# naver/dust3r

Measured on NVIDIA H100. Metric: image-pairs/sec (512x384, ViT-L/B+DPT), higher is better.
Workload: dtype bf16

## Files before the change

### dust3r_b200/_lib.py

```python
from __future__ import annotations

import ctypes as C
import os

from ._lib_fwd import Model

_HERE = os.path.dirname(os.path.abspath(__file__))
LIB_PATH = os.path.join(_HERE, 'libdust3r_b200.so')

_lib = None


class D3RError(RuntimeError):
    pass


class AlignDesc(C.Structure):
    _fields_ = [
        ('n_imgs', C.c_int32), ('n_edges', C.c_int32), ('n_entries', C.c_int32), ('n_chunks', C.c_int32),
        ('max_deg', C.c_int32), ('max_chunks', C.c_int32), ('chunk_px', C.c_int32), ('dist_l2', C.c_int32), ('norm_pw_scale', C.c_int32),
        ('tied_focal', C.c_int32), ('eval_only', C.c_int32),
        ('base_scale', C.c_float), ('pw_break', C.c_float), ('focal_break', C.c_float), ('adam_eps', C.c_float),
        ('beta1', C.c_float), ('beta2', C.c_float),
        ('img_hw', C.c_void_p), ('img_pix_off', C.c_void_p), ('img_ent_ptr', C.c_void_p),
        ('img_chunk_ptr', C.c_void_p), ('chunk_img', C.c_void_p),
        ('ent_edge', C.c_void_p), ('ent_obs_off', C.c_void_p), ('ent_coef', C.c_void_p), ('edge_ent', C.c_void_p),
        ('obs', C.c_void_p),
        ('logd', C.c_void_p), ('logd_m', C.c_void_p), ('logd_v', C.c_void_p),
        ('small', C.c_void_p), ('small_m', C.c_void_p), ('small_v', C.c_void_p), ('small_trainable', C.c_void_p),
        ('workspace', C.c_void_p), ('sched', C.c_void_p), ('loss_out', C.c_void_p), ('counters', C.c_void_p),
        ('stream_kernel', C.c_int32), ('stream_grid', C.c_int32), ('stream_ppt', C.c_int32), ('stream_window', C.c_int32),
        ('n_items', C.c_int32), ('reserved0', C.c_int32), ('items', C.c_void_p), ('warp_item_ptr', C.c_void_p),
        ('items_rev', C.c_void_p), ('warp_item_ptr_rev', C.c_void_p),
    ]


class JpegHuff(C.Structure):
    _fields_ = [('maxcode', C.c_int32 * 18), ('valoff', C.c_int32 * 18), ('look', C.c_uint16 * 512), ('val', C.c_uint8 * 256)]


class JpegDesc(C.Structure):
    _fields_ = [
        ('width', C.c_int32), ('height', C.c_int32), ('n_comp', C.c_int32), ('restart_interval', C.c_int32),
        ('orientation', C.c_int32), ('reserved', C.c_int32), ('scan_begin', C.c_int64),
        ('h_samp', C.c_int32 * 3), ('v_samp', C.c_int32 * 3), ('dc_table', C.c_int32 * 3), ('ac_table', C.c_int32 * 3),
        ('quant', (C.c_uint16 * 64) * 3), ('huff', JpegHuff * 8),
    ]


class PngDesc(C.Structure):
    _fields_ = [
        ('width', C.c_int32), ('height', C.c_int32), ('color_type', C.c_int32), ('orientation', C.c_int32),
        ('palette_len', C.c_int32), ('reserved', C.c_int32), ('idat_bytes', C.c_int64), ('palette', (C.c_uint8 * 3) * 256),
    ]


class ViewDesc(C.Structure):
    _fields_ = [
        ('src', C.c_void_p), ('depth', C.c_void_p), ('src_pitch', C.c_int32), ('depth_pitch', C.c_int32),
        ('H0', C.c_int32), ('W0', C.c_int32), ('H1', C.c_int32), ('W1', C.c_int32), ('crop_x0', C.c_int32), ('crop_y0', C.c_int32),
        ('H2', C.c_int32), ('W2', C.c_int32), ('row0', C.c_int32), ('rows', C.c_int32), ('transpose', C.c_int32),
        ('reserved', C.c_int32), ('xbounds', C.c_void_p), ('xcoefs', C.c_void_p), ('ybounds', C.c_void_p), ('ycoefs', C.c_void_p),
        ('fu', C.c_float), ('fv', C.c_float), ('cu', C.c_float), ('cv', C.c_float), ('pose', C.c_float * 12),
        ('tmp', C.c_void_p), ('img', C.c_void_p), ('depthmap', C.c_void_p), ('pts3d', C.c_void_p), ('valid', C.c_void_p),
        ('blocks', C.c_int64 * 3),
    ]


vp, i32, i64, u32, f32, f64 = C.c_void_p, C.c_int32, C.c_int64, C.c_uint32, C.c_float, C.c_double
_DESC, _MODEL, _JPEG, _PNG, _VIEW = (C.POINTER(AlignDesc), C.POINTER(Model), C.POINTER(JpegDesc), C.POINTER(PngDesc),
                                     C.POINTER(ViewDesc))

PROTOTYPES = {
    'd3r_last_error': (C.c_char_p, []),
    'd3r_abi_version': (i32, []),
    'd3r_check_device': (i32, []),
    'd3r_launch_count': (i64, []),
    'd3r_launch_count_reset': (None, []),
    'd3r_prof_enable': (None, [i32]),
    'd3r_prof_report': (i32, [C.c_char_p, i32]),
    'd3r_prof_dump': (i32, [C.c_char_p, i32]),
    'd3r_sizeof_align_desc': (i32, []),
    'd3r_sizeof_align_item': (i32, []),
    'd3r_align_chunk_pixels': (i32, []),
    'd3r_align_workspace_floats': (i64, [i32, i32]),
    'd3r_align_prepare': (i32, [_DESC, vp]),
    'd3r_align_run': (i32, [_DESC, i32, i32, vp]),
    'd3r_align_pixel_pass': (i32, [_DESC, i32, vp]),
    'd3r_align_small_step': (i32, [_DESC, i32, vp]),
    'd3r_align_reduce_block': (i32, [i32, i32, C.POINTER(i64), C.POINTER(i64)]),
    'd3r_align_grad_pixel_pass': (i32, [_DESC, vp, vp]),
    'd3r_align_grad_small_step': (i32, [_DESC, vp, vp, vp]),
    'd3r_align_loss_grad': (i32, [_DESC, vp, vp, vp, vp]),
    'd3r_align_overflow_flag': (i32, [_DESC, C.POINTER(i32), vp]),
    'd3r_align_pts3d': (i32, [_DESC, vp, vp]),
    'd3r_align_set_debug': (i32, [vp]),
    'd3r_sizeof_pack_entry': (i32, []),
    'd3r_align_stream_slots_per_item': (i32, []),
    'd3r_align_stream_warps_per_cta': (i32, []),
    'd3r_align_stream_max_window': (i32, []),
    'd3r_align_pack_entries': (i32, [vp, i32, i32, i32, i32, vp, vp]),
    'd3r_gemm_bf16': (i32, [vp, vp, vp, vp, vp, vp, i32, i32, i32, i64, u32, vp, vp, i32, i32, i32, vp]),
    'd3r_conv3x3_bf16': (i32, [vp, vp, vp, vp, vp, vp, vp, i32, i32, i32, i32, i32, u32, vp]),
    'd3r_attention_hd64': (i32, [vp, i64, vp, i64, vp, i64, vp, i64, i32, i32, i32, i32, f32, vp]),
    'd3r_conv_transpose_bf16': (i32, [vp, vp, vp, vp, i32, i32, i32, i32, i32, i32, vp]),
    'd3r_conv3x3_head_tail': (i32, [vp, vp, vp, vp, vp, vp, vp, i32, i32, i32, i32, i32, f32, f32, vp]),
    'd3r_layernorm_bf16': (i32, [vp, vp, vp, vp, i32, i32, f32, vp]),
    'd3r_upsample2x_bf16': (i32, [vp, vp, i32, i32, i32, i32, i32, i32, vp]),
    'd3r_im2col_3x3_s2_bf16': (i32, [vp, vp, i32, i32, i32, i32, vp]),
    'd3r_patch_im2col16': (i32, [vp, vp, i32, i32, i32, vp]),
    'd3r_linear_head_postprocess': (i32, [vp, vp, vp, i32, i32, i32, i32, i32, i32, f32, f32, vp]),
    'd3r_set_gemm_impl': (None, [i32]),
    'd3r_set_gemm_store': (None, [i32]),
    'd3r_set_conv_store': (None, [i32]),
    'd3r_set_attention_impl': (None, [i32]),
    'd3r_clean_pointcloud': (i32, [i32, vp, vp, i32, vp, vp, vp, vp, vp, f32, f32, vp]),
    'd3r_procrustes_moments': (i32, [i32, i32, vp, vp, vp, vp, vp]),
    'd3r_weiszfeld_focal': (i32, [i32, i32, i32, vp, vp, i32, vp, vp]),
    'd3r_nearest_neighbours': (i32, [i32, i32, vp, vp, vp, vp]),
    'd3r_image_resize_crop_normalize': (i32, [vp, i32, i32, i32, i32, vp, vp, i32, vp, vp, i32, i32, i32, i32, i32, i32, i32,
                                              vp, vp, vp, vp]),
    'd3r_sizeof_view_desc': (i32, []),
    'd3r_prepare_views': (i32, [i32, _VIEW, vp, vp, vp]),
    'd3r_sizeof_jpeg_desc': (i32, []),
    'd3r_jpeg_decode_workspace_bytes': (i64, [_JPEG, i64]),
    'd3r_jpeg_decode': (i32, [_JPEG, vp, i64, vp, vp, vp, i64, vp]),
    'd3r_sizeof_png_desc': (i32, []),
    'd3r_png_decode_workspace_bytes': (i64, [_PNG, i64]),
    'd3r_png_decode': (i32, [_PNG, vp, i64, vp, vp, vp, i64, vp]),
    'd3r_segment_sky_workspace_bytes': (i64, [i32, i64]),
    'd3r_segment_sky': (i32, [i32, vp, vp, i32, i64, vp, vp, vp, i64, vp]),
    'd3r_nanmedian_workspace_bytes': (i64, [i32]),
    'd3r_segmented_nanmedian': (i32, [i32, i64, vp, vp, vp, i64, vp]),
    'd3r_criterion_workspace_bytes': (i64, [i32, i64, i64, i32]),
    'd3r_criterion': (i32, [i32, i64, i64, i32, i32, f32, f32] + [vp] * 15 + [i64, vp]),
    'd3r_pnp_ransac_workspace_bytes': (i64, [i32]),
    'd3r_pnp_ransac': (i32, [i32, vp, vp, f64, f64, f64, f64, f64, f64, i32, i64, vp, i64, vp, vp, vp, vp]),
    'd3r_pnp_hypotheses': (i32, [i32, vp, vp, f64, f64, f64, f64, f64, i64, i32, i32, vp, vp, vp, vp]),
    'd3r_sizeof_model': (i32, []),
    'd3r_encode_workspace_bytes': (i64, [_MODEL, i32, i32, i32]),
    'd3r_encode_images': (i32, [_MODEL, vp, i32, i32, i32, vp, vp, i64, vp]),
    'd3r_decode_workspace_bytes': (i64, [_MODEL, i32, i32, i32, i32, i32]),
    'd3r_decode_pairs': (i32, [_MODEL, vp, i32, i32, i32, vp, i32, i32, i32, C.POINTER(i32), C.POINTER(i32), i32,
                               vp, vp, vp, vp, vp, i64, vp]),
    'd3r_forward_set_debug': (i32, [i32, vp, i64]),
}


def lib_available() -> bool:
    return os.path.exists(LIB_PATH)


def get_lib():
    global _lib
    if _lib is None:
        if not os.path.exists(LIB_PATH):
            raise D3RError(f'{LIB_PATH} not found: the CUDA extension is required (no CPU/torch fallback). '
                           f'Build it with `python -m dust3r_b200.build`.')
        lib = C.CDLL(LIB_PATH)
        for name, (restype, argtypes) in PROTOTYPES.items():
            fn = getattr(lib, name)
            fn.restype, fn.argtypes = restype, argtypes
        _lib = lib
    return _lib


def check(rc: int):
    if rc != 0:
        msg = get_lib().d3r_last_error().decode(errors='replace')
        raise D3RError(f'dust3r_b200 error {rc}: {msg}')


def require_cuda_device(device):
    import torch
    dev = torch.device(device)
    if dev.type != 'cuda':
        raise D3RError(f'dust3r_b200 computes on CUDA sm_90a only (got device {dev}); there is no CPU fallback')
    if not torch.cuda.is_available():
        raise D3RError('CUDA is not available: dust3r_b200 has no CPU fallback')
    with torch.cuda.device(dev):
        check(get_lib().d3r_check_device())
    return dev


def cuda_device(device):
    import torch
    dev = require_cuda_device(device)
    return torch.device('cuda', torch.cuda.current_device()) if dev.index is None else dev


def launch(device, name, *args):
    import torch
    with torch.cuda.device(device):
        check(getattr(get_lib(), name)(*args, C.c_void_p(torch.cuda.current_stream(device).cuda_stream)))


def stream_ptr():
    import torch
    return C.c_void_p(torch.cuda.current_stream().cuda_stream)


def launch_count(reset=False):
    lib = get_lib()
    n = int(lib.d3r_launch_count())
    if reset:
        lib.d3r_launch_count_reset()
    return n


def prof_enable(on=True):
    get_lib().d3r_prof_enable(1 if on else 0)


def prof_report():
    import json
    buf = C.create_string_buffer(1 << 16)
    n = get_lib().d3r_prof_report(buf, len(buf))
    if n < 0:
        raise D3RError('profile report does not fit the buffer')
    return json.loads(buf.value.decode())


def prof_dump():
    import json
    buf = C.create_string_buffer(1 << 22)
    n = get_lib().d3r_prof_dump(buf, len(buf))
    if n < 0:
        raise D3RError('profile dump does not fit the buffer')
    return json.loads(buf.value.decode())
```

### dust3r_b200/csrc/c_api.cu

```cuda
#include "d3r_common.cuh"
#include <cstring>
#include <mutex>

namespace d3r {

static thread_local char g_err[1024] = "";

void set_error(const char* fmt, ...) {
  va_list ap;
  va_start(ap, fmt);
  vsnprintf(g_err, sizeof(g_err), fmt, ap);
  va_end(ap);
}

int num_sms() {
  static int sms = 0;
  if (sms == 0) {
    int dev = 0;
    cudaGetDevice(&dev);
    cudaDeviceGetAttribute(&sms, cudaDevAttrMultiProcessorCount, dev);
    if (sms <= 0) sms = 132;
  }
  return sms;
}

typedef CUresult (*EncodeTiledFn)(CUtensorMap*, CUtensorMapDataType, cuuint32_t, void*, const cuuint64_t*, const cuuint64_t*,
                                  const cuuint32_t*, const cuuint32_t*, CUtensorMapInterleave, CUtensorMapSwizzle,
                                  CUtensorMapL2promotion, CUtensorMapFloatOOBfill);

int encode_tensor_map(CUtensorMap* m, const void* base, int rank, const cuuint64_t* dims, const cuuint64_t* strides_bytes,
                      const cuuint32_t* box, const char* op, CUtensorMapDataType dtype) {
  static EncodeTiledFn fn = nullptr;
  static std::once_flag once;
  std::call_once(once, [] {
    void* p = nullptr;
    cudaDriverEntryPointQueryResult q;
    if (cudaGetDriverEntryPoint("cuTensorMapEncodeTiled", &p, cudaEnableDefault, &q) == cudaSuccess && q == cudaDriverEntryPointSuccess)
      fn = reinterpret_cast<EncodeTiledFn>(p);
  });
  if (!fn) {
    set_error("%s: cuTensorMapEncodeTiled is not available from the CUDA driver", op);
    return D3R_ERR_CUDA;
  }
  const cuuint32_t estr[5] = {1, 1, 1, 1, 1};
  CUresult r = fn(m, dtype, (cuuint32_t)rank, const_cast<void*>(base), dims, strides_bytes, box, estr,
                  CU_TENSOR_MAP_INTERLEAVE_NONE, CU_TENSOR_MAP_SWIZZLE_128B, CU_TENSOR_MAP_L2_PROMOTION_L2_256B,
                  CU_TENSOR_MAP_FLOAT_OOB_FILL_NONE);
  if (r != CUDA_SUCCESS) {
    set_error("%s: cuTensorMapEncodeTiled failed with CUresult %d (rank %d, dims %llu,%llu)", op, (int)r, rank,
              (unsigned long long)dims[0], (unsigned long long)dims[1]);
    return D3R_ERR_CUDA;
  }
  return D3R_OK;
}

}

extern "C" const char* d3r_last_error(void) { return d3r::g_err; }

extern "C" int d3r_abi_version(void) { return 6; }

extern "C" int d3r_check_device(void) {
  int dev = 0;
  D3R_CUDA(cudaGetDevice(&dev));
  int major = 0, minor = 0;
  D3R_CUDA(cudaDeviceGetAttribute(&major, cudaDevAttrComputeCapabilityMajor, dev));
  D3R_CUDA(cudaDeviceGetAttribute(&minor, cudaDevAttrComputeCapabilityMinor, dev));
  if (major != 9 || minor != 0) {
    d3r::set_error("dust3r_b200 is built for sm_90a only; device %d is sm_%d%d", dev, major, minor);
    return D3R_ERR_UNSUPPORTED_DEVICE;
  }
  return D3R_OK;
}
```

### dust3r_b200/csrc/d3r_common.cuh

```cuda
#pragma once
#include <cuda.h>
#include <cuda_runtime.h>
#include <cuda_bf16.h>
#include <cstdint>
#include <cstdio>
#include <cstdarg>

#include "../../include/dust3r_b200.h"

namespace d3r {

void set_error(const char* fmt, ...);

#define D3R_CHECK_ARG(cond, ...)                    \
  do {                                              \
    if (!(cond)) {                                  \
      ::d3r::set_error(__VA_ARGS__);                \
      return D3R_ERR_INVALID;                       \
    }                                               \
  } while (0)

#define D3R_CUDA(expr)                                                                     \
  do {                                                                                     \
    cudaError_t _e = (expr);                                                               \
    if (_e != cudaSuccess) {                                                               \
      ::d3r::set_error("%s failed: %s (%s:%d)", #expr, cudaGetErrorString(_e), __FILE__, __LINE__); \
      return D3R_ERR_CUDA;                                                                 \
    }                                                                                      \
  } while (0)

#define D3R_LAUNCH_CHECK()                                                                 \
  do {                                                                                     \
    cudaError_t _e = cudaGetLastError();                                                   \
    if (_e != cudaSuccess) {                                                               \
      ::d3r::set_error("kernel launch failed: %s (%s:%d)", cudaGetErrorString(_e), __FILE__, __LINE__); \
      return D3R_ERR_CUDA;                                                                 \
    }                                                                                      \
  } while (0)

__device__ __forceinline__ float warp_sum(float v) {
  v += __shfl_xor_sync(0xffffffffu, v, 16);
  v += __shfl_xor_sync(0xffffffffu, v, 8);
  v += __shfl_xor_sync(0xffffffffu, v, 4);
  v += __shfl_xor_sync(0xffffffffu, v, 2);
  v += __shfl_xor_sync(0xffffffffu, v, 1);
  return v;
}

__device__ __forceinline__ uint32_t pack_bf16x2(float a, float b) {
  __nv_bfloat162 h = __floats2bfloat162_rn(a, b);
  return *reinterpret_cast<uint32_t*>(&h);
}
__device__ __forceinline__ float2 bf16x2_to_float2(uint32_t w) {
  const __nv_bfloat162 h = *reinterpret_cast<const __nv_bfloat162*>(&w);
  return make_float2(__low2float(h), __high2float(h));
}

template <class ConfIn>
__device__ __forceinline__ void postprocess_pixel(float x, float y, float z, ConfIn conf_in, float* pts3d, float* conf, long long pix,
                                                  int depth_mode, int conf_mode, float cmin, float cmax) {
  float ox = x, oy = y, oz = z;
  if (depth_mode != 0) {
    const float d = sqrtf(x * x + y * y + z * z);
    const float dc = fmaxf(d, 1e-8f);
    const float s = (depth_mode == 2) ? expm1f(d) : d * d;
    ox = x / dc * s; oy = y / dc * s; oz = z / dc * s;
  }
  float* o = pts3d + pix * 3;
  o[0] = ox; o[1] = oy; o[2] = oz;
  if (conf_mode != 0) {
    const float c = conf_in();
    float r;
    if (conf_mode == 1) r = cmin + fminf(expf(c), cmax - cmin);
    else r = (cmax - cmin) * (1.f / (1.f + expf(-c))) + cmin;
    conf[pix] = r;
  }
}

int num_sms();

int encode_tensor_map(CUtensorMap* m, const void* base, int rank, const cuuint64_t* dims, const cuuint64_t* strides_bytes,
                      const cuuint32_t* box, const char* op, CUtensorMapDataType dtype = CU_TENSOR_MAP_DATA_TYPE_BFLOAT16);

inline bool first_launch_on_this_device(unsigned long long& mask) {
  int dev = 0;
  cudaGetDevice(&dev);
  const unsigned long long bit = 1ull << (dev & 63);
  if (mask & bit) return false;
  mask |= bit;
  return true;
}

}
```

### dust3r_b200/csrc/forward.cu

```cuda
#include "gemm_host.h"
#include "elementwise.h"
#include <vector>
#include <cstring>

namespace d3r {
namespace fwd {

using gemm::Params;

struct Arena {
  uint8_t* base;
  size_t cap, off;
  bool dry;
  void* take(size_t bytes) {
    off = (off + 255) & ~size_t(255);
    void* p = dry ? nullptr : base + off;
    off += bytes;
    return p;
  }
  template <class T>
  T* arr(size_t n) { return reinterpret_cast<T*>(take(n * sizeof(T))); }
};

struct DebugTap { int stage; float* out; long long cap; };
static thread_local DebugTap g_tap = {-1, nullptr, 0};

__global__ void bf16_to_f32_kernel(const __nv_bfloat16* x, float* o, size_t n) {
  size_t i = (size_t)blockIdx.x * blockDim.x + threadIdx.x;
  if (i < n) o[i] = __bfloat162float(x[i]);
}
static void tap_f32(int stage, const float* x, size_t n, cudaStream_t st) {
  if (g_tap.stage == stage && g_tap.out && (long long)n <= g_tap.cap)
    cudaMemcpyAsync(g_tap.out, x, n * sizeof(float), cudaMemcpyDeviceToDevice, st);
}
static void tap_bf16(int stage, const void* x, size_t n, cudaStream_t st) {
  if (g_tap.stage == stage && g_tap.out && (long long)n <= g_tap.cap)
    bf16_to_f32_kernel<<<(unsigned)((n + 255) / 256), 256, 0, st>>>((const __nv_bfloat16*)x, g_tap.out, n);
}

#define RC(x)            \
  do {                   \
    int _rc = (x);       \
    if (_rc) return _rc; \
  } while (0)

struct Ctx {
  const d3r_model* m;
  cudaStream_t st;
  int gh, gw, N;
};

static int linear(const Ctx& c, const void* A, long long lda, const d3r_linear& w, int M, int N, int K, void* out, uint32_t flags,
                  void* out2 = nullptr, const void* add0 = nullptr, int rope_cols = 0) {
  Params p{};
  p.M = M; p.N = N; p.K = K;
  p.flags = flags | (w.b ? gemm::F_BIAS : 0);
  p.out = out; p.out2 = out2; p.add0 = add0; p.bias = w.b; p.ldo = N;
  if (flags & gemm::F_ROPE) {
    p.rope_cos = c.m->rope_cos; p.rope_sin = c.m->rope_sin; p.rope_cols = rope_cols; p.tokens_per_img = c.N; p.grid_w = c.gw;
  }
  return gemm::gemm_bf16(A, lda, w.w, p, c.st);
}

static int conv3(const Ctx& c, const void* x, const d3r_linear& w, int B, int H, int W, int Cin, int Cout, void* out, uint32_t flags,
                 const void* add0 = nullptr, const void* add1 = nullptr, void* out2 = nullptr) {
  Params p{};
  p.flags = flags | (w.b ? gemm::F_BIAS : 0) | (add0 ? gemm::F_ADD0 : 0) | (add1 ? gemm::F_ADD1 : 0) | (out2 ? gemm::F_OUT2_RELU : 0);
  p.out = out; p.out2 = out2; p.add0 = add0; p.add1 = add1; p.bias = w.b;
  return gemm::conv3x3_bf16(x, w.w, B, H, W, Cin, Cout, p, c.st);
}

static int run_encoder(const Ctx& c, Arena& ar, const float* imgs, int n_enc, int H, int W, __nv_bfloat16* eout) {
  const d3r_model& m = *c.m;
  const int E = m.enc_dim, M = n_enc * c.N, hid = E * m.mlp_ratio, pk = 3 * m.patch * m.patch;
  float* x = ar.arr<float>((size_t)M * E);
  __nv_bfloat16* ln = ar.arr<__nv_bfloat16>((size_t)M * E);
  __nv_bfloat16* qkv = ar.arr<__nv_bfloat16>((size_t)M * 3 * E);
  __nv_bfloat16* att = ar.arr<__nv_bfloat16>((size_t)M * E);
  __nv_bfloat16* hidb = ar.arr<__nv_bfloat16>((size_t)M * (hid > pk ? hid : pk));
  if (ar.dry) return D3R_OK;
  RC(ew::patch_im2col16(imgs, hidb, n_enc, H, W, c.st));
  RC(linear(c, hidb, pk, m.patch_embed, M, E, pk, x, gemm::F_OUT_F32));
  tap_f32(1, x, (size_t)M * E, c.st);
  const float scale = 1.0f / sqrtf(float(E / m.enc_heads));
  for (int l = 0; l < m.enc_depth; ++l) {
    const d3r_enc_block& b = m.enc[l];
    RC(ew::layernorm(x, b.norm1.g, b.norm1.b, ln, nullptr, M, E, m.ln_eps, c.st));
    RC(linear(c, ln, E, b.qkv, M, 3 * E, E, qkv, gemm::F_ROPE, nullptr, nullptr, 2 * E));
    RC(attn::attention_hd64(qkv, 3 * E, qkv + E, 3 * E, qkv + 2 * E, 3 * E, att, E, n_enc, m.enc_heads, c.N, c.N, scale, c.st));
    RC(linear(c, att, E, b.proj, M, E, E, x, gemm::F_RESID_INPLACE));
    RC(ew::layernorm(x, b.norm2.g, b.norm2.b, ln, nullptr, M, E, m.ln_eps, c.st));
    RC(linear(c, ln, E, b.fc1, M, hid, E, hidb, gemm::F_GELU));
    RC(linear(c, hidb, hid, b.fc2, M, E, hid, x, gemm::F_RESID_INPLACE));
    if (l == 0) tap_f32(2, x, (size_t)M * E, c.st);
  }
  tap_f32(3, x, (size_t)M * E, c.st);
  RC(ew::layernorm(x, m.enc_norm.g, m.enc_norm.b, eout, nullptr, M, E, m.ln_eps, c.st));
  tap_bf16(4, eout, (size_t)M * E, c.st);
  return D3R_OK;
}

struct DecBufs {
  __nv_bfloat16 *ln, *qkv, *att, *q, *kv, *hid;
};
static int dec_block(const Ctx& c, const Ctx& cy, const d3r_dec_block& b, float* x, const __nv_bfloat16* ynorm, const DecBufs& w,
                     int B) {
  const d3r_model& m = *c.m;
  const int D = m.dec_dim, M = B * c.N, My = B * cy.N, hid = D * m.mlp_ratio;
  const float scale = 1.0f / sqrtf(float(D / m.dec_heads));
  RC(ew::layernorm(x, b.norm1.g, b.norm1.b, w.ln, nullptr, M, D, m.ln_eps, c.st));
  RC(linear(c, w.ln, D, b.qkv, M, 3 * D, D, w.qkv, gemm::F_ROPE, nullptr, nullptr, 2 * D));
  RC(attn::attention_hd64(w.qkv, 3 * D, w.qkv + D, 3 * D, w.qkv + 2 * D, 3 * D, w.att, D, B, m.dec_heads, c.N, c.N, scale, c.st));
  RC(linear(c, w.att, D, b.proj, M, D, D, x, gemm::F_RESID_INPLACE));
  RC(ew::layernorm(x, b.norm2.g, b.norm2.b, w.ln, nullptr, M, D, m.ln_eps, c.st));
  RC(linear(c, w.ln, D, b.projq, M, D, D, w.q, gemm::F_ROPE, nullptr, nullptr, D));
  RC(linear(cy, ynorm, D, b.projkv, My, 2 * D, D, w.kv, gemm::F_ROPE, nullptr, nullptr, D));
  RC(attn::attention_hd64(w.q, D, w.kv, 2 * D, w.kv + D, 2 * D, w.att, D, B, m.dec_heads, c.N, cy.N, scale, c.st));
  RC(linear(c, w.att, D, b.cproj, M, D, D, x, gemm::F_RESID_INPLACE));
  RC(ew::layernorm(x, b.norm3.g, b.norm3.b, w.ln, nullptr, M, D, m.ln_eps, c.st));
  RC(linear(c, w.ln, D, b.fc1, M, hid, D, w.hid, gemm::F_GELU));
  RC(linear(c, w.hid, hid, b.fc2, M, D, hid, x, gemm::F_RESID_INPLACE));
  return D3R_OK;
}

static int run_dpt(const Ctx& c, Arena& ar, const d3r_dpt_head& hd, const void* const tok[4], int B, float* pts3d, float* conf) {
  const d3r_model& m = *c.m;
  const int gh = c.gh, gw = c.gw, F = 256;
  const int dims[4] = {m.enc_dim, m.dec_dim, m.dec_dim, m.dec_dim};
  const int ld[4] = {96, 192, 384, 768};
  const int Mt = B * c.N;
  const int h3 = (gh - 1) / 2 + 1, w3 = (gw - 1) / 2 + 1;
  const int Hs[4] = {gh * 4, gh * 2, gh, h3}, Ws[4] = {gw * 4, gw * 2, gw, w3};
  typedef __nv_bfloat16 bf;
  bf* a0 = ar.arr<bf>((size_t)Mt * 96);
  bf* a1 = ar.arr<bf>((size_t)Mt * 192);
  bf* a3 = ar.arr<bf>((size_t)Mt * 768);
  bf* l[4];
  l[0] = ar.arr<bf>((size_t)B * Hs[0] * Ws[0] * 96);
  l[1] = ar.arr<bf>((size_t)B * Hs[1] * Ws[1] * 192);
  l[2] = ar.arr<bf>((size_t)Mt * 384);
  l[3] = ar.arr<bf>((size_t)B * h3 * w3 * 768);
  bf* col = ar.arr<bf>((size_t)B * h3 * w3 * 9 * 768);
  bf *r[4], *rr[4];
  for (int k = 0; k < 4; ++k) {
    r[k] = ar.arr<bf>((size_t)B * Hs[k] * Ws[k] * F);
    rr[k] = ar.arr<bf>((size_t)B * Hs[k] * Ws[k] * F);
  }
  const size_t big = (size_t)B * Hs[0] * Ws[0] * F;
  bf* t = ar.arr<bf>(big);
  bf* s = ar.arr<bf>(big);
  bf* sr = ar.arr<bf>(big);
  bf* y = ar.arr<bf>(big);
  bf* z = ar.arr<bf>(big);
  bf* path = ar.arr<bf>(big * 4);
  const int Hf = gh * 16, Wf = gw * 16;
  bf* h0 = ar.arr<bf>((size_t)B * (Hf / 2) * (Wf / 2) * 128);
  bf* h1 = ar.arr<bf>((size_t)B * Hf * Wf * 128);
  if (ar.dry) return D3R_OK;

  RC(linear(c, tok[0], dims[0], hd.act_conv[0], Mt, ld[0], dims[0], a0, 0));
  RC(gemm::conv_transpose_bf16(a0, hd.act0_up.w, l[0], hd.act0_up.b, B, gh, gw, 96, 96, 4, c.st));
  RC(linear(c, tok[1], dims[1], hd.act_conv[1], Mt, ld[1], dims[1], a1, 0));
  RC(gemm::conv_transpose_bf16(a1, hd.act1_up.w, l[1], hd.act1_up.b, B, gh, gw, 192, 192, 2, c.st));
  RC(linear(c, tok[2], dims[2], hd.act_conv[2], Mt, ld[2], dims[2], l[2], 0));
  RC(linear(c, tok[3], dims[3], hd.act_conv[3], Mt, ld[3], dims[3], a3, 0));
  RC(ew::im2col_3x3_s2_bf16(a3, col, B, gh, gw, 768, c.st));
  RC(linear(c, col, 9 * 768, hd.act3_down, B * h3 * w3, 768, 9 * 768, l[3], 0));
  for (int k = 0; k < 4; ++k) RC(conv3(c, l[k], hd.layer_rn[k], B, Hs[k], Ws[k], ld[k], F, r[k], 0, nullptr, nullptr, rr[k]));
  tap_bf16(20, r[0], (size_t)B * Hs[0] * Ws[0] * F, c.st);
  tap_bf16(23, r[3], (size_t)B * Hs[3] * Ws[3] * F, c.st);

  const bf* prev_path = nullptr;
  for (int lvl = 3; lvl >= 0; --lvl) {
    const d3r_fusion& f = hd.refine[lvl];
    const int Hc = Hs[lvl], Wc = Ws[lvl];
    const bf *sum_raw, *sum_relu;
    if (lvl == 3) {
      sum_raw = r[3];
      sum_relu = rr[3];
    } else {
      RC(conv3(c, rr[lvl], f.rcu1_conv1, B, Hc, Wc, F, F, t, gemm::F_RELU));
      RC(conv3(c, t, f.rcu1_conv2, B, Hc, Wc, F, F, s, 0, r[lvl], prev_path, sr));
      sum_raw = s;
      sum_relu = sr;
    }
    RC(conv3(c, sum_relu, f.rcu2_conv1, B, Hc, Wc, F, F, t, gemm::F_RELU));
    RC(conv3(c, t, f.rcu2_conv2, B, Hc, Wc, F, F, y, 0, sum_raw));
    RC(linear(c, y, F, f.out_conv, B * Hc * Wc, F, F, z, 0));
    const int Ho = (lvl == 3) ? Hs[2] : 2 * Hc, Wo = (lvl == 3) ? Ws[2] : 2 * Wc;
    RC(ew::upsample2x_bf16(z, path, B, Hc, Wc, F, Ho, Wo, c.st));
    prev_path = path;
    if (lvl == 3) tap_bf16(24, path, (size_t)B * Ho * Wo * F, c.st);
    if (lvl == 0) tap_bf16(21, path, (size_t)B * Ho * Wo * F, c.st);
  }
  const int Hp = Hs[0] * 2, Wp = Ws[0] * 2;
  RC(conv3(c, path, hd.head0, B, Hp, Wp, F, 128, h0, 0));
  RC(ew::upsample2x_bf16(h0, h1, B, Hp, Wp, 128, Hf, Wf, c.st));
  RC(gemm::conv3x3_head_tail(h1, hd.head2.w, hd.head2.b, hd.head4_w, hd.head4_b, pts3d, conf, B, Hf, Wf, m.depth_mode,
                             (m.nch > 3 && conf) ? m.conf_mode : 0, m.conf_min, m.conf_max, c.st));
  return D3R_OK;
}

static int decode_heads(const d3r_model* mp, const Ctx cv[2], const void* const enc[2], const int32_t* const maps_host[2], int B,
                        float* pts1, float* conf1, float* pts2, float* conf2, Arena& ar, cudaStream_t st) {
  const d3r_model& m = *mp;
  const int E = m.enc_dim, D = m.dec_dim, hid = D * m.mlp_ratio;
  const int Md[2] = {B * cv[0].N, B * cv[1].N};
  const int Mx = Md[0] > Md[1] ? Md[0] : Md[1];
  typedef __nv_bfloat16 bf;

  bf* f[2];
  f[0] = ar.arr<bf>((size_t)Md[0] * E);
  f[1] = ar.arr<bf>((size_t)Md[1] * E);
  int* maps = ar.arr<int>((size_t)2 * B);
  float* x[2] = {ar.arr<float>((size_t)Md[0] * D), ar.arr<float>((size_t)Md[1] * D)};
  bf* yn[2] = {ar.arr<bf>((size_t)Md[1] * D), ar.arr<bf>((size_t)Md[0] * D)};
  DecBufs w;
  w.ln = ar.arr<bf>((size_t)Mx * D);
  w.qkv = ar.arr<bf>((size_t)Mx * 3 * D);
  w.att = ar.arr<bf>((size_t)Mx * D);
  w.q = ar.arr<bf>((size_t)Mx * D);
  w.kv = ar.arr<bf>((size_t)Mx * 2 * D);
  w.hid = ar.arr<bf>((size_t)Mx * hid);
  bf* hook[2][3];
  for (int br = 0; br < 2; ++br)
    for (int k = 0; k < 3; ++k) hook[br][k] = ar.arr<bf>((size_t)Md[br] * D);
  float* lin_feat = nullptr;
  if (m.head_type == 0) lin_feat = ar.arr<float>((size_t)Mx * m.nch * m.patch * m.patch);

  const size_t mark_head = ar.off;
  if (m.head_type == 1) {
    size_t top = ar.off;
    for (int br = 0; br < 2; ++br) {
      Arena probe = ar;
      const void* none[4] = {nullptr, nullptr, nullptr, nullptr};
      probe.dry = true;
      RC(run_dpt(cv[br], probe, *m.dpt[br], none, B, nullptr, nullptr));
      if (probe.off > top) top = probe.off;
    }
    if (ar.dry) ar.off = top;
  }
  if (ar.dry) return D3R_OK;

  if (ar.off > ar.cap && m.head_type != 1) {
    set_error("forward: workspace too small (%zu > %zu bytes)", ar.off, ar.cap);
    return D3R_ERR_INVALID;
  }

  for (int br = 0; br < 2; ++br) {
    D3R_CUDA(cudaMemcpyAsync(maps + br * B, maps_host[br], sizeof(int) * B, cudaMemcpyHostToDevice, st));
    RC(ew::gather_images_bf16(enc[br], f[br], maps + br * B, B, cv[br].N, E, st));
  }

  RC(linear(cv[0], f[0], E, m.decoder_embed, Md[0], D, E, x[0], gemm::F_OUT_F32));
  RC(linear(cv[1], f[1], E, m.decoder_embed, Md[1], D, E, x[1], gemm::F_OUT_F32));
  tap_f32(5, x[0], (size_t)Md[0] * D, st);
  for (int l = 0; l < m.dec_depth; ++l) {
    RC(ew::layernorm(x[1], m.dec1[l].norm_y.g, m.dec1[l].norm_y.b, yn[0], nullptr, Md[1], D, m.ln_eps, st));
    RC(ew::layernorm(x[0], m.dec2[l].norm_y.g, m.dec2[l].norm_y.b, yn[1], nullptr, Md[0], D, m.ln_eps, st));
    RC(dec_block(cv[0], cv[1], m.dec1[l], x[0], yn[0], w, B));
    RC(dec_block(cv[1], cv[0], m.dec2[l], x[1], yn[1], w, B));
    if (l == 0) { tap_f32(6, x[0], (size_t)Md[0] * D, st); tap_f32(7, x[1], (size_t)Md[1] * D, st); }
    for (int k = 1; k <= 2; ++k) {
      if (m.head_type == 1 && l + 1 == m.hooks[k]) {
        RC(ew::cast_f32_bf16(x[0], hook[0][k - 1], (size_t)Md[0] * D, st));
        RC(ew::cast_f32_bf16(x[1], hook[1][k - 1], (size_t)Md[1] * D, st));
      }
    }
  }
  tap_f32(8, x[0], (size_t)Md[0] * D, st);
  tap_f32(9, x[1], (size_t)Md[1] * D, st);
  RC(ew::layernorm(x[0], m.dec_norm.g, m.dec_norm.b, hook[0][2], nullptr, Md[0], D, m.ln_eps, st));
  RC(ew::layernorm(x[1], m.dec_norm.g, m.dec_norm.b, hook[1][2], nullptr, Md[1], D, m.ln_eps, st));

  float* outs[2][2] = {{pts1, conf1}, {pts2, conf2}};
  if (m.head_type == 0) {
    const int nf = m.nch * m.patch * m.patch;
    for (int br = 0; br < 2; ++br) {
      RC(linear(cv[br], hook[br][2], D, m.lin_head[br], Md[br], nf, D, lin_feat, gemm::F_OUT_F32));
      RC(ew::linear_head_postprocess(lin_feat, outs[br][0], outs[br][1], B, cv[br].gh, cv[br].gw, m.nch, m.depth_mode, m.conf_mode,
                                     m.conf_min, m.conf_max, st));
    }
  } else {
    for (int br = 0; br < 2; ++br) {
      Arena head = ar;
      head.off = mark_head;
      const void* tok[4] = {f[br], hook[br][0], hook[br][1], hook[br][2]};
      RC(run_dpt(cv[br], head, *m.dpt[br], tok, B, outs[br][0], outs[br][1]));
      if (head.off > head.cap) {
        set_error("forward: workspace too small (%zu > %zu bytes)", head.off, head.cap);
        return D3R_ERR_INVALID;
      }
    }
  }
  return D3R_OK;
}

static Ctx token_grid(const d3r_model* mp, cudaStream_t st, int H, int W) {
  return Ctx{mp, st, H / mp->patch, W / mp->patch, (H / mp->patch) * (W / mp->patch)};
}

static int encode(const d3r_model* mp, const float* imgs, int n, int H, int W, void* feat, Arena& ar, cudaStream_t st) {
  return run_encoder(token_grid(mp, st, H, W), ar, imgs, n, H, W, reinterpret_cast<__nv_bfloat16*>(feat));
}

static int decode(const d3r_model* mp, const void* feat1, int H1, int W1, const void* feat2, int H2, int W2, const int32_t* idx1,
                  const int32_t* idx2, int B, float* pts1, float* conf1, float* pts2, float* conf2, Arena& ar, cudaStream_t st) {
  const Ctx cv[2] = {token_grid(mp, st, H1, W1), token_grid(mp, st, H2, W2)};
  const void* enc[2] = {feat1, feat2};
  const int32_t* maps[2] = {idx1, idx2};
  return decode_heads(mp, cv, enc, maps, B, pts1, conf1, pts2, conf2, ar, st);
}

}
}

using namespace d3r;

static bool aligned16(const void* p) { return (reinterpret_cast<uintptr_t>(p) & 15) == 0; }

static int check_model(const d3r_model* m, int H, int W) {
  D3R_CHECK_ARG(m != nullptr, "forward: null model");
  D3R_CHECK_ARG(m->patch == 16, "forward: patch size %d unsupported (16 only)", m->patch);
  D3R_CHECK_ARG(m->enc_dim % 64 == 0 && m->enc_dim / m->enc_heads == 64, "forward: encoder head dim must be 64");
  D3R_CHECK_ARG(m->dec_dim % 64 == 0 && m->dec_dim / m->dec_heads == 64, "forward: decoder head dim must be 64");
  D3R_CHECK_ARG(H > 0 && W > 0 && H % 16 == 0 && W % 16 == 0, "forward: image %dx%d is not a multiple of the patch size", H, W);
  D3R_CHECK_ARG(m->rope_cos && m->rope_sin && m->rope_max_pos >= (H > W ? H : W) / 16, "forward: RoPE tables too small");
  D3R_CHECK_ARG(m->head_type == 0 || m->head_type == 1, "forward: bad head type");
  D3R_CHECK_ARG(m->head_type == 0 || (m->enc_dim % 32 == 0 && m->dpt[0] && m->dpt[1]), "forward: missing DPT weights");
  return D3R_OK;
}

extern "C" int64_t d3r_encode_workspace_bytes(const d3r_model* m, int32_t n, int32_t H, int32_t W) {
  if (check_model(m, H, W)) return -1;
  if (n <= 0) {
    set_error("encode: empty batch (n=%d)", n);
    return -1;
  }
  fwd::Arena ar{nullptr, 0, 0, true};
  if (fwd::encode(m, nullptr, n, H, W, nullptr, ar, 0)) return -1;
  return (int64_t)ar.off + 4096;
}

extern "C" int d3r_encode_images(const d3r_model* m, const float* imgs_dev, int32_t n, int32_t H, int32_t W, void* feat_dev,
                                 void* workspace_dev, int64_t workspace_bytes, void* stream) {
  RC(check_model(m, H, W));
  D3R_CHECK_ARG(imgs_dev && feat_dev && workspace_dev, "encode: null buffer");
  D3R_CHECK_ARG(n > 0, "encode: empty batch (n=%d)", n);
  D3R_CHECK_ARG(aligned16(imgs_dev) && aligned16(feat_dev), "encode: images and features must be 16-byte aligned");
  const int64_t need = d3r_encode_workspace_bytes(m, n, H, W);
  D3R_CHECK_ARG(need > 0 && workspace_bytes >= need, "encode: workspace of %lld bytes needed, %lld given", (long long)need,
                (long long)workspace_bytes);
  fwd::Arena ar{reinterpret_cast<uint8_t*>(workspace_dev), (size_t)workspace_bytes, 0, false};
  const int rc = fwd::encode(m, imgs_dev, n, H, W, feat_dev, ar, (cudaStream_t)stream);
  fwd::g_tap = {-1, nullptr, 0};
  return rc;
}

extern "C" int64_t d3r_decode_workspace_bytes(const d3r_model* m, int32_t B, int32_t H1, int32_t W1, int32_t H2, int32_t W2) {
  if (check_model(m, H1, W1) || check_model(m, H2, W2)) return -1;
  if (B <= 0) {
    set_error("decode: empty batch (B=%d)", B);
    return -1;
  }
  fwd::Arena ar{nullptr, 0, 0, true};
  if (fwd::decode(m, nullptr, H1, W1, nullptr, H2, W2, nullptr, nullptr, B, nullptr, nullptr, nullptr, nullptr, ar, 0)) return -1;
  return (int64_t)ar.off + 4096;
}

extern "C" int d3r_decode_pairs(const d3r_model* m, const void* feat1_dev, int32_t n1, int32_t H1, int32_t W1, const void* feat2_dev,
                                int32_t n2, int32_t H2, int32_t W2, const int32_t* idx1_host, const int32_t* idx2_host, int32_t B,
                                float* pts3d_1, float* conf_1, float* pts3d_2, float* conf_2, void* workspace_dev,
                                int64_t workspace_bytes, void* stream) {
  RC(check_model(m, H1, W1));
  RC(check_model(m, H2, W2));
  D3R_CHECK_ARG(feat1_dev && feat2_dev && idx1_host && idx2_host && pts3d_1 && pts3d_2 && workspace_dev, "decode: null buffer");
  D3R_CHECK_ARG(n1 > 0 && n2 > 0 && B > 0, "decode: empty batch (n1=%d, n2=%d, B=%d)", n1, n2, B);
  D3R_CHECK_ARG(aligned16(feat1_dev) && aligned16(feat2_dev), "decode: features must be 16-byte aligned");
  D3R_CHECK_ARG(feat1_dev != feat2_dev || (n1 == n2 && H1 == H2 && W1 == W2),
                "decode: one feature buffer given with two sizes (%d x %dx%d, %d x %dx%d)", n1, H1, W1, n2, H2, W2);
  for (int b = 0; b < B; ++b)
    D3R_CHECK_ARG(idx1_host[b] >= 0 && idx1_host[b] < n1 && idx2_host[b] >= 0 && idx2_host[b] < n2,
                  "decode: pair %d indexes images (%d, %d) of (%d, %d)", b, idx1_host[b], idx2_host[b], n1, n2);
  const int64_t need = d3r_decode_workspace_bytes(m, B, H1, W1, H2, W2);
  D3R_CHECK_ARG(need > 0 && workspace_bytes >= need, "decode: workspace of %lld bytes needed, %lld given", (long long)need,
                (long long)workspace_bytes);
  fwd::Arena ar{reinterpret_cast<uint8_t*>(workspace_dev), (size_t)workspace_bytes, 0, false};
  const int rc = fwd::decode(m, feat1_dev, H1, W1, feat2_dev, H2, W2, idx1_host, idx2_host, B, pts3d_1, conf_1, pts3d_2, conf_2, ar,
                             (cudaStream_t)stream);
  fwd::g_tap = {-1, nullptr, 0};
  return rc;
}

extern "C" int d3r_sizeof_model(void) { return (int)sizeof(d3r_model); }

extern "C" int d3r_forward_set_debug(int32_t stage_id, float* out_dev, int64_t capacity_floats) {
  fwd::g_tap = {stage_id, out_dev, capacity_floats};
  return D3R_OK;
}
```

### dust3r_b200/csrc/gemm_host.cu

```cuda
#include "gemm_wgmma.cuh"
#include "gemm_host.h"
#include "prof.h"

namespace d3r {
namespace gemm {

static int pick_block_n(int N, int mode, uint32_t flags, int conv_m_tiles = 0) {
  if (flags & F_HEAD_FINAL) return 128;
  if (conv_m_tiles > 0) return (N == 256 && (conv_m_tiles + 1) / 2 >= 4 * (num_sms() / 2)) ? 256 : 128;
  if (N % 256 == 0 && pick_epi(mode, flags) != EPI_GENERIC) return 256;
  if (N % 128 == 0) return 128;
  if (N % 64 == 0) return 64;
  return (N > 128) ? 128 : 64;
}

static int g_impl = 2;
constexpr int kPairMinKb = 4;
static bool use_pair(int bn, int num_kb) { return bn >= 128 && (g_impl == 1 || (g_impl == 2 && num_kb >= kPairMinKb)); }

static int g_store = 1;
static int g_conv_store = 1;

static int grid_for(bool pair, int m_tiles, int n_tiles) {
  if (pair) {
    const int items = ((m_tiles + 1) / 2) * n_tiles;
    const int max_clusters = num_sms() / 2;
    return 2 * (items < max_clusters ? items : max_clusters);
  }
  const int items = m_tiles * n_tiles;
  return items < num_sms() ? items : num_sms();
}

static const char* prof_tag(const Params& p, int bn, bool pair) {
  return (p.mode == 1) ? ((p.flags & F_HEAD_FINAL) ? (pair ? "conv3x3_head_tail_2cta" : "conv3x3_head_tail")
                                                   : (pair ? "conv3x3_wgmma_2cta" : "conv3x3_wgmma"))
                       : (bn == 256 ? (pair ? "gemm_wgmma_2cta_bn256" : "gemm_wgmma_bn256")
                                    : (pair ? "gemm_wgmma_2cta_bn128" : (bn == 128 ? "gemm_wgmma_bn128" : "gemm_wgmma_bn64")));
}

template <int BN, int EPI, bool PAIR, bool TMA_STORE = false>
static int launch(const CUtensorMap& ta, const CUtensorMap& tb, const CUtensorMap& to, const Params& p, int m_tiles, int n_tiles,
                  cudaStream_t st) {
  constexpr int kSmem = Cfg<BN, TMA_STORE>::kSmemBytes;
  static unsigned long long attr_devices = 0;
  if (first_launch_on_this_device(attr_devices))
    D3R_CUDA(cudaFuncSetAttribute(gemm_kernel<BN, EPI, PAIR, TMA_STORE>, cudaFuncAttributeMaxDynamicSharedMemorySize, kSmem));
  const int grid = grid_for(PAIR, m_tiles, n_tiles);
  char detail[96];
  snprintf(detail, sizeof(detail), "M=%d N=%d K=%d flags=0x%x mode=%d epi=%d", p.M, p.N, p.K, (unsigned)p.flags, p.mode, EPI);
  prof::Scope scope(prof_tag(p, BN, PAIR), st, 2.0 * double(p.M) * double(p.N) * double(p.K), 0.0, 1, detail);
  D3R_CUDA(pdl::launch_clustered(gemm_kernel<BN, EPI, PAIR, TMA_STORE>, dim3(grid), dim3(kNumThreads), size_t(kSmem), st, PAIR ? 2 : 1,
                                 ta, tb, to, p));
  D3R_LAUNCH_CHECK();
  return D3R_OK;
}

template <int BN, bool PAIR>
static int launch_conv(const CUtensorMap& ta, const CUtensorMap& tb, const CUtensorMap& to, const ConvMaps& cm, const Params& p,
                       int m_tiles, int n_tiles, cudaStream_t st) {
  constexpr int kSmem = Cfg<BN, true>::kSmemBytes;
  static unsigned long long attr_devices = 0;
  if (first_launch_on_this_device(attr_devices))
    D3R_CUDA(cudaFuncSetAttribute(conv_kernel<BN, PAIR>, cudaFuncAttributeMaxDynamicSharedMemorySize, kSmem));
  const int grid = grid_for(PAIR, m_tiles, n_tiles);
  char detail[96];
  snprintf(detail, sizeof(detail), "M=%d N=%d K=%d flags=0x%x mode=%d epi=%d", p.M, p.N, p.K, (unsigned)p.flags, p.mode, EPI_GENERIC);
  prof::Scope scope(prof_tag(p, BN, PAIR), st, 2.0 * double(p.M) * double(p.N) * double(p.K), 0.0, 1, detail);
  D3R_CUDA(pdl::launch_clustered(conv_kernel<BN, PAIR>, dim3(grid), dim3(kNumThreads), size_t(kSmem), st, PAIR ? 2 : 1, ta, tb, to, cm, p));
  D3R_LAUNCH_CHECK();
  return D3R_OK;
}

template <int BN, bool PAIR>
static int dispatch_epi(int epi, const CUtensorMap& ta, const CUtensorMap& tb, const CUtensorMap* to, const Params& p, int m_tiles,
                        int n_tiles, cudaStream_t st) {
  if constexpr (BN == 256) {
    if (to) {
      switch (epi) {
        case EPI_RESID: return launch<BN, EPI_RESID, PAIR, true>(ta, tb, *to, p, m_tiles, n_tiles, st);
        case EPI_ACT: return launch<BN, EPI_ACT, PAIR, true>(ta, tb, *to, p, m_tiles, n_tiles, st);
        case EPI_ROPE: return launch<BN, EPI_ROPE, PAIR, true>(ta, tb, *to, p, m_tiles, n_tiles, st);
      }
    }
  }
  switch (epi) {
    case EPI_RESID: return launch<BN, EPI_RESID, PAIR>(ta, tb, tb, p, m_tiles, n_tiles, st);
    case EPI_ACT: return launch<BN, EPI_ACT, PAIR>(ta, tb, tb, p, m_tiles, n_tiles, st);
    case EPI_ROPE: return launch<BN, EPI_ROPE, PAIR>(ta, tb, tb, p, m_tiles, n_tiles, st);
  }
  if constexpr (BN == 128) return launch<128, EPI_GENERIC, PAIR>(ta, tb, tb, p, m_tiles, n_tiles, st);
  set_error("no BLOCK_N %d kernel for the generic epilogue", BN);
  return D3R_ERR_INVALID;
}

static int dispatch(int bn, const CUtensorMap& ta, const CUtensorMap& tb, const CUtensorMap* to, const Params& p, int m_tiles,
                    cudaStream_t st) {
  const int n_tiles = (p.N + bn - 1) / bn;
  const int epi = (bn >= 128) ? pick_epi(p.mode, p.flags) : EPI_GENERIC;
  const bool pair = use_pair(bn, p.num_kb);
  switch (bn) {
    case 256: return pair ? dispatch_epi<256, true>(epi, ta, tb, to, p, m_tiles, n_tiles, st) : dispatch_epi<256, false>(epi, ta, tb, to, p, m_tiles, n_tiles, st);
    case 128: return pair ? dispatch_epi<128, true>(epi, ta, tb, nullptr, p, m_tiles, n_tiles, st) : dispatch_epi<128, false>(epi, ta, tb, nullptr, p, m_tiles, n_tiles, st);
    case 64: return launch<64, EPI_GENERIC, false>(ta, tb, tb, p, m_tiles, n_tiles, st);
  }
  set_error("unsupported BLOCK_N %d", bn);
  return D3R_ERR_INVALID;
}

static int make_tmap_b(CUtensorMap* m, const void* B, int N, int taps, int Kc, int bn, int num_kb, const char* op) {
  cuuint64_t dims[3] = {(cuuint64_t)Kc, (cuuint64_t)taps, (cuuint64_t)N};
  cuuint64_t str[2] = {(cuuint64_t)Kc * 2, (cuuint64_t)taps * Kc * 2};
  cuuint32_t box[3] = {(cuuint32_t)BLOCK_K, 1, (cuuint32_t)(use_pair(bn, num_kb) ? bn / 2 : bn)};
  return encode_tensor_map(m, B, 3, dims, str, box, op);
}

int gemm_bf16(const void* A, long long lda, const void* B, Params p, cudaStream_t st) {
  D3R_CHECK_ARG(A && B, "gemm: null operand");
  D3R_CHECK_ARG(p.M > 0 && p.N > 0 && p.K > 0, "gemm: bad shape %d %d %d", p.M, p.N, p.K);
  D3R_CHECK_ARG(p.N % 32 == 0, "gemm: N=%d must be a multiple of 32", p.N);
  D3R_CHECK_ARG(p.K % 8 == 0 && lda % 8 == 0, "gemm: K=%d / lda=%lld must be multiples of 8 (16-byte TMA strides)", p.K, lda);
  D3R_CHECK_ARG((reinterpret_cast<uintptr_t>(A) & 15) == 0 && (reinterpret_cast<uintptr_t>(B) & 15) == 0, "gemm: operands must be 16-byte aligned");
  p.mode = 0;
  p.num_kb = (p.K + BLOCK_K - 1) / BLOCK_K;
  const int bn = pick_block_n(p.N, p.mode, p.flags);
  CUtensorMap ta, tb;
  {
    cuuint64_t dims[2] = {(cuuint64_t)p.K, (cuuint64_t)p.M};
    cuuint64_t str[1] = {(cuuint64_t)lda * 2};
    cuuint32_t box[2] = {(cuuint32_t)BLOCK_K, (cuuint32_t)BLOCK_M};
    int rc = encode_tensor_map(&ta, A, 2, dims, str, box, "gemm");
    if (rc) return rc;
  }
  int rc = make_tmap_b(&tb, B, p.N, 1, p.K, bn, p.num_kb, "gemm");
  if (rc) return rc;
  CUtensorMap to;
  const bool f32 = (p.flags & F_RESID_INPLACE) != 0;
  const long long row_bytes = p.ldo * (f32 ? 4 : 2);
  const bool staged = g_store == 1 && bn == 256 && pick_epi(p.mode, p.flags) != EPI_GENERIC && p.ldo >= p.N && row_bytes % 16 == 0 &&
                      (reinterpret_cast<uintptr_t>(p.out) & 15) == 0;
  if (staged) {
    cuuint64_t dims[2] = {(cuuint64_t)p.N, (cuuint64_t)p.M};
    cuuint64_t str[1] = {(cuuint64_t)row_bytes};
    cuuint32_t box[2] = {(cuuint32_t)(f32 ? 32 : 64), 64};
    rc = encode_tensor_map(&to, p.out, 2, dims, str, box, "gemm output", f32 ? CU_TENSOR_MAP_DATA_TYPE_FLOAT32 : CU_TENSOR_MAP_DATA_TYPE_BFLOAT16);
    if (rc) return rc;
  }
  return dispatch(bn, ta, tb, staged ? &to : nullptr, p, (p.M + BLOCK_M - 1) / BLOCK_M, st);
}

static int make_tmap_conv_io(CUtensorMap* m, const void* base, int B, int H, int W, int C, int tile_w, const char* op) {
  const int bw = tile_w < 64 ? tile_w : 64;
  cuuint64_t dims[4] = {(cuuint64_t)C, (cuuint64_t)W, (cuuint64_t)H, (cuuint64_t)B};
  cuuint64_t str[3] = {(cuuint64_t)C * 2, (cuuint64_t)W * C * 2, (cuuint64_t)H * W * C * 2};
  cuuint32_t box[4] = {64, (cuuint32_t)bw, (cuuint32_t)(64 / bw), 1};
  return encode_tensor_map(m, base, 4, dims, str, box, op);
}

static bool aligned16(const void* ptr) { return (reinterpret_cast<uintptr_t>(ptr) & 15) == 0; }

int conv3x3_bf16(const void* x_nhwc, const void* w_packed, int B, int H, int W, int Cin, int Cout, Params p, cudaStream_t st) {
  D3R_CHECK_ARG(x_nhwc && w_packed, "conv3x3: null operand");
  D3R_CHECK_ARG(Cin % 8 == 0 && Cout % 32 == 0, "conv3x3: Cin=%d must be a multiple of 8 and Cout=%d of 32", Cin, Cout);
  p.mode = 1;
  p.M = B * H * W;
  p.N = Cout;
  p.cin_blocks = (Cin + BLOCK_K - 1) / BLOCK_K;
  p.K = 9 * Cin;
  p.num_kb = 9 * p.cin_blocks;
  p.cB = B; p.cH = H; p.cW = W;
  int tw = 16;
  while (tw < W && tw < 128) tw *= 2;
  p.tile_w = tw;
  p.tile_h = BLOCK_M / tw;
  p.tiles_x = (W + p.tile_w - 1) / p.tile_w;
  p.tiles_y = (H + p.tile_h - 1) / p.tile_h;
  p.ldo = Cout;
  const int m_tiles = B * p.tiles_x * p.tiles_y;
  const bool staged = g_conv_store == 1 && (Cout == 256 || Cout == 128) && (p.flags & ~EpiMask<EPI_CONV>::value) == 0 &&
                      aligned16(p.out) && (!(p.flags & F_OUT2_RELU) || aligned16(p.out2)) && (!(p.flags & F_ADD0) || aligned16(p.add0)) &&
                      (!(p.flags & F_ADD1) || aligned16(p.add1));
  const int bn = pick_block_n(p.N, p.mode, p.flags, staged ? m_tiles : 0);
  CUtensorMap ta, tb;
  {
    cuuint64_t dims[4] = {(cuuint64_t)Cin, (cuuint64_t)W, (cuuint64_t)H, (cuuint64_t)B};
    cuuint64_t str[3] = {(cuuint64_t)Cin * 2, (cuuint64_t)W * Cin * 2, (cuuint64_t)H * W * Cin * 2};
    cuuint32_t box[4] = {(cuuint32_t)BLOCK_K, (cuuint32_t)p.tile_w, (cuuint32_t)p.tile_h, 1};
    int rc = encode_tensor_map(&ta, x_nhwc, 4, dims, str, box, "conv3x3");
    if (rc) return rc;
  }
  int rc = make_tmap_b(&tb, w_packed, Cout, 9, Cin, bn, p.num_kb, "conv3x3");
  if (rc) return rc;
  if (!staged) return dispatch(bn, ta, tb, nullptr, p, m_tiles, st);
  CUtensorMap to;
  ConvMaps cm;
  rc = make_tmap_conv_io(&to, p.out, B, H, W, Cout, p.tile_w, "conv3x3 output");
  if (rc) return rc;
  cm.out2 = cm.add0 = cm.add1 = to;
  const struct { uint32_t flag; const void* base; CUtensorMap* map; const char* op; } io[3] = {
      {F_OUT2_RELU, p.out2, &cm.out2, "conv3x3 out2"}, {F_ADD0, p.add0, &cm.add0, "conv3x3 add0"}, {F_ADD1, p.add1, &cm.add1, "conv3x3 add1"}};
  for (const auto& t : io) {
    if (!(p.flags & t.flag)) continue;
    rc = make_tmap_conv_io(t.map, t.base, B, H, W, Cout, p.tile_w, t.op);
    if (rc) return rc;
  }
  const int n_tiles = Cout / bn;
  const bool pair = use_pair(bn, p.num_kb);
  if (bn == 256) return pair ? launch_conv<256, true>(ta, tb, to, cm, p, m_tiles, n_tiles, st) : launch_conv<256, false>(ta, tb, to, cm, p, m_tiles, n_tiles, st);
  return pair ? launch_conv<128, true>(ta, tb, to, cm, p, m_tiles, n_tiles, st) : launch_conv<128, false>(ta, tb, to, cm, p, m_tiles, n_tiles, st);
}

int conv_transpose_bf16(const void* x_nhwc, const void* w_packed, void* out, const float* bias, int B, int h, int w, int Cin, int Cout,
                        int k, cudaStream_t st) {
  D3R_CHECK_ARG(x_nhwc && w_packed && out, "conv_transpose: null buffer");
  D3R_CHECK_ARG(B > 0 && h > 0 && w > 0 && Cin > 0 && Cout > 0 && k > 0, "conv_transpose: bad shape B=%d h=%d w=%d Cin=%d Cout=%d k=%d", B,
                h, w, Cin, Cout, k);
  D3R_CHECK_ARG(Cin % 8 == 0, "conv_transpose: Cin=%d must be a multiple of 8", Cin);
  D3R_CHECK_ARG(Cout % 2 == 0 && (k * k * Cout) % 32 == 0, "conv_transpose: Cout=%d must be even and k*k*Cout=%d a multiple of 32", Cout,
                k * k * Cout);
  Params p{};
  p.M = B * h * w; p.N = k * k * Cout; p.K = Cin;
  p.flags = F_CONVT | (bias ? F_BIAS : 0);
  p.out = out; p.bias = bias; p.ldo = 0;
  p.tk = k; p.th_in = h; p.tw_in = w; p.tCout = Cout;
  return gemm_bf16(x_nhwc, Cin, w_packed, p, st);
}

int conv3x3_head_tail(const void* x_nhwc, const void* w_packed, const float* bias, const float* w4, const float* b4, float* pts3d,
                      float* conf, int B, int H, int W, int depth_mode, int conf_mode, float conf_min, float conf_max, cudaStream_t st) {
  D3R_CHECK_ARG(x_nhwc && w_packed && w4 && b4 && pts3d, "conv3x3_head_tail: null buffer");
  D3R_CHECK_ARG(B > 0 && H > 0 && W > 0, "conv3x3_head_tail: bad shape B=%d H=%d W=%d", B, H, W);
  D3R_CHECK_ARG(depth_mode >= 0 && depth_mode <= 2, "conv3x3_head_tail: depth_mode %d out of range", depth_mode);
  D3R_CHECK_ARG(conf_mode >= 0 && conf_mode <= 2, "conv3x3_head_tail: conf_mode %d out of range", conf_mode);
  D3R_CHECK_ARG(conf_mode == 0 || conf, "conv3x3_head_tail: conf_mode %d without a conf buffer", conf_mode);
  Params p{};
  p.flags = F_HEAD_FINAL | (bias ? F_BIAS : 0);
  p.bias = bias;
  p.w4 = w4; p.b4 = b4;
  p.pts3d = pts3d; p.conf = conf;
  p.depth_mode = depth_mode; p.conf_mode = conf_mode;
  p.conf_min = conf_min; p.conf_max = conf_max;
  return conv3x3_bf16(x_nhwc, w_packed, B, H, W, 128, 128, p, st);
}

}
}

using namespace d3r;

extern "C" void d3r_set_gemm_impl(int32_t impl) { gemm::g_impl = impl; }
extern "C" void d3r_set_gemm_store(int32_t store) { gemm::g_store = store; }
extern "C" void d3r_set_conv_store(int32_t store) { gemm::g_conv_store = store; }

extern "C" int d3r_gemm_bf16(const void* A, const void* B, void* out, const float* bias, const void* add0, void* out2,
                             int32_t M, int32_t N, int32_t K, int64_t ldo, uint32_t flags, const float* rope_cos,
                             const float* rope_sin, int32_t rope_cols, int32_t tokens_per_img, int32_t grid_w, void* stream) {
  gemm::Params p{};
  p.M = M; p.N = N; p.K = K;
  p.flags = flags;
  p.out = out; p.out2 = out2; p.add0 = add0; p.bias = bias; p.ldo = ldo;
  p.rope_cos = rope_cos; p.rope_sin = rope_sin; p.rope_cols = rope_cols; p.tokens_per_img = tokens_per_img; p.grid_w = grid_w;
  D3R_CHECK_ARG(!(flags & gemm::F_BIAS) || bias, "gemm: F_BIAS without bias");
  D3R_CHECK_ARG(!(flags & gemm::F_ROPE) || (rope_cos && rope_sin && tokens_per_img > 0 && grid_w > 0), "gemm: F_ROPE without tables");
  D3R_CHECK_ARG(!(flags & (gemm::F_CONVT | gemm::F_HEAD_FINAL)),
                "gemm: F_CONVT / F_HEAD_FINAL have their own entry points, d3r_conv_transpose_bf16 / d3r_conv3x3_head_tail");
  return gemm::gemm_bf16(A, K, B, p, (cudaStream_t)stream);
}

extern "C" int d3r_conv3x3_bf16(const void* x_nhwc, const void* w_packed, void* out, const float* bias, const void* add0,
                                const void* add1, void* out2, int32_t B, int32_t H, int32_t W, int32_t Cin, int32_t Cout,
                                uint32_t flags, void* stream) {
  gemm::Params p{};
  p.flags = flags;
  p.out = out; p.out2 = out2; p.add0 = add0; p.add1 = add1; p.bias = bias;
  D3R_CHECK_ARG(!(flags & (gemm::F_CONVT | gemm::F_HEAD_FINAL | gemm::F_ROPE)), "conv3x3: unsupported flag");
  return gemm::conv3x3_bf16(x_nhwc, w_packed, B, H, W, Cin, Cout, p, (cudaStream_t)stream);
}

extern "C" int d3r_conv_transpose_bf16(const void* x_nhwc, const void* w_packed, void* out, const float* bias, int32_t B, int32_t h,
                                       int32_t w, int32_t Cin, int32_t Cout, int32_t k, void* stream) {
  return gemm::conv_transpose_bf16(x_nhwc, w_packed, out, bias, B, h, w, Cin, Cout, k, (cudaStream_t)stream);
}

extern "C" int d3r_conv3x3_head_tail(const void* x_nhwc, const void* w_packed, const float* bias, const float* w4, const float* b4,
                                     float* pts3d, float* conf, int32_t B, int32_t H, int32_t W, int32_t depth_mode, int32_t conf_mode,
                                     float conf_min, float conf_max, void* stream) {
  return gemm::conv3x3_head_tail(x_nhwc, w_packed, bias, w4, b4, pts3d, conf, B, H, W, depth_mode, conf_mode, conf_min, conf_max,
                                 (cudaStream_t)stream);
}
```

### dust3r_b200/csrc/gemm_host.h

```cpp
#pragma once
#include "gemm_wgmma.cuh"

namespace d3r {
namespace gemm {
int gemm_bf16(const void* A, long long lda, const void* B, Params p, cudaStream_t st);
int conv3x3_bf16(const void* x_nhwc, const void* w_packed, int B, int H, int W, int Cin, int Cout, Params p, cudaStream_t st);
int conv_transpose_bf16(const void* x_nhwc, const void* w_packed, void* out, const float* bias, int B, int h, int w, int Cin, int Cout,
                        int k, cudaStream_t st);
int conv3x3_head_tail(const void* x_nhwc, const void* w_packed, const float* bias, const float* w4, const float* b4, float* pts3d,
                      float* conf, int B, int H, int W, int depth_mode, int conf_mode, float conf_min, float conf_max, cudaStream_t st);
}
}
```

### dust3r_b200/csrc/gemm_wgmma.cuh

```cuda
#pragma once
#include "d3r_common.cuh"
#include "sm90_ptx.cuh"
#include "pdl.cuh"

namespace d3r {
namespace gemm {

constexpr int BLOCK_M = 128;
constexpr int BLOCK_K = 64;
constexpr int WGMMA_K = 16;
constexpr int kNumThreads = 384;
constexpr int kConsumerWarps = 8;

enum : uint32_t {
  F_BIAS = 1u << 0,
  F_GELU = 1u << 1,
  F_RELU = 1u << 2,
  F_OUT_F32 = 1u << 3,
  F_RESID_INPLACE = 1u << 4,
  F_ADD0 = 1u << 5,
  F_ADD1 = 1u << 6,
  F_OUT2_RELU = 1u << 7,
  F_ROPE = 1u << 8,
  F_CONVT = 1u << 9,
  F_HEAD_FINAL = 1u << 10,
  F_OUT2_BF16 = 1u << 11,
};

struct Params {
  int M, N, K;
  int num_kb;
  int mode;
  uint32_t flags;
  void* out;
  void* out2;
  const void* add0;
  const void* add1;
  const float* bias;
  long long ldo;
  const float* rope_cos;
  const float* rope_sin;
  int rope_cols, tokens_per_img, grid_w;
  int cB, cH, cW, cin_blocks, tile_w, tile_h, tiles_x, tiles_y;
  int tk, th_in, tw_in, tCout;
  const float* w4;
  const float* b4;
  float* pts3d;
  float* conf;
  int depth_mode;
  int conf_mode;
  float conf_min, conf_max;
};

enum : int { EPI_GENERIC = 0, EPI_RESID = 1, EPI_ACT = 2, EPI_ROPE = 3, EPI_CONV = 4 };
template <int EPI> struct EpiMask { static constexpr uint32_t value = 0xFFFFFFFFu; };
template <> struct EpiMask<EPI_RESID> { static constexpr uint32_t value = F_BIAS | F_RESID_INPLACE; };
template <> struct EpiMask<EPI_ACT> { static constexpr uint32_t value = F_BIAS | F_GELU | F_RELU; };
template <> struct EpiMask<EPI_ROPE> { static constexpr uint32_t value = F_BIAS | F_ROPE; };
template <> struct EpiMask<EPI_CONV> { static constexpr uint32_t value = F_BIAS | F_RELU | F_ADD0 | F_ADD1 | F_OUT2_RELU; };

struct ConvMaps {
  CUtensorMap out2, add0, add1;
};

__host__ __device__ inline int pick_epi(int mode, uint32_t flags) {
  if (mode != 0) return EPI_GENERIC;
  if ((flags & ~F_BIAS) == F_RESID_INPLACE) return EPI_RESID;
  if ((flags & ~EpiMask<EPI_ACT>::value) == 0) return EPI_ACT;
  if ((flags & ~EpiMask<EPI_ROPE>::value) == 0) return EPI_ROPE;
  return EPI_GENERIC;
}

template <int BLOCK_N, bool TMA_STORE = false>
struct Cfg {
  static constexpr int kStageA = BLOCK_M * BLOCK_K * 2;
  static constexpr int kStageB = BLOCK_N * BLOCK_K * 2;
  static constexpr int kStages = (BLOCK_N == 256) ? 4 : (BLOCK_N == 128) ? 6 : 8;
  static constexpr int kRing = kStages * (kStageA + kStageB);
  static constexpr int kOutBuf = 64 * 128;
  static constexpr int kStaging = TMA_STORE ? 2 * 2 * kOutBuf : 0;
  static constexpr int kSmemBytes = kRing + kStaging + 1024  + 256  + (TMA_STORE ? 0 : (4 * 128 + 16) * 4) ;
  static_assert(kSmemBytes <= 227 * 1024, "shared memory of one CTA");
};

__device__ __forceinline__ float gelu_erf(float x) {
  constexpr float kU = 0.84932180028801904f;
  constexpr float kP = 0.3275911f * 0.70710678118654752f / kU;
  const float u = fabsf(x) * kU;
  const float t = ptx::rcp_approx(fmaf(kP, u, 1.f));
  float poly = fmaf(0.5f * 1.061405429f, t, 0.5f * -1.453152027f);
  poly = fmaf(poly, t, 0.5f * 1.421413741f);
  poly = fmaf(poly, t, 0.5f * -0.284496736f);
  poly = fmaf(poly, t, 0.5f * 0.254829592f);
  const float e = ptx::ex2_approx(-u * u);
  const float h = x * (poly * t * e);
  return fmaxf(x, 0.f) - fabsf(h);
}

template <int BLOCK_N, int EPI, bool PAIR, bool TMA_STORE>
__device__ __forceinline__ void gemm_body(const CUtensorMap& tmap_a, const CUtensorMap& tmap_b, const CUtensorMap& tmap_o,
                                          const ConvMaps* cm, const Params& p) {
  static_assert(EPI == EPI_CONV ? (TMA_STORE && (BLOCK_N == 256 || BLOCK_N == 128))
                                : (!TMA_STORE || (BLOCK_N == 256 && EPI != EPI_GENERIC)),
                "TMA-store epilogue: specialised projection epilogues on 128x256 tiles, the conv epilogue on 128x256 / 128x128");
  using C = Cfg<BLOCK_N, TMA_STORE>;
  extern __shared__ uint8_t smem_raw[];
  uint8_t* smem = reinterpret_cast<uint8_t*>((reinterpret_cast<uintptr_t>(smem_raw) + 1023) & ~uintptr_t(1023));
  uint8_t* smem_a = smem;
  uint8_t* smem_b = smem + C::kStages * C::kStageA;
  uint8_t* smem_o = smem + C::kRing;
  uint64_t* bars = reinterpret_cast<uint64_t*>(smem + C::kRing + C::kStaging);
  uint64_t* full_bar = bars;
  uint64_t* empty_bar = bars + C::kStages;
  uint64_t* add_bar = bars + 2 * C::kStages;
  float* s_w4 = reinterpret_cast<float*>(reinterpret_cast<uint8_t*>(bars) + 256);

  const int warp = threadIdx.x >> 5, lane = threadIdx.x & 31;
  const uint32_t rank = PAIR ? ptx::cluster_ctarank() : 0u;
  const int n_tiles = (p.N + BLOCK_N - 1) / BLOCK_N;
  const int m_tiles = (p.mode == 1) ? p.cB * p.tiles_y * p.tiles_x : (p.M + BLOCK_M - 1) / BLOCK_M;
  const int m_groups = PAIR ? (m_tiles + 1) / 2 : m_tiles;
  const int total_items = m_groups * n_tiles;
  const int first_item = PAIR ? blockIdx.x / 2 : blockIdx.x;
  const int item_stride = PAIR ? gridDim.x / 2 : gridDim.x;

  if (threadIdx.x == 0) {
    ptx::prefetch_tmap(&tmap_a);
    ptx::prefetch_tmap(&tmap_b);
    if constexpr (TMA_STORE) ptx::prefetch_tmap(&tmap_o);
    for (int s = 0; s < C::kStages; ++s) {
      ptx::mbar_init(ptx::smem_u32(&full_bar[s]), 1);
      ptx::mbar_init(ptx::smem_u32(&empty_bar[s]), (PAIR ? 2 : 1) * kConsumerWarps);
    }
    if constexpr (EPI == EPI_CONV) {
      ptx::prefetch_tmap(&cm->out2);
      ptx::prefetch_tmap(&cm->add0);
      ptx::prefetch_tmap(&cm->add1);
      ptx::mbar_init(ptx::smem_u32(&add_bar[0]), 1);
      ptx::mbar_init(ptx::smem_u32(&add_bar[1]), 1);
    }
    ptx::fence_barrier_init();
  }
  if (!TMA_STORE && (p.flags & F_HEAD_FINAL) && threadIdx.x >= 128) {
    for (int i = threadIdx.x - 128; i < 4 * 128 + 4; i += 256) s_w4[i] = (i < 512) ? p.w4[i] : p.b4[i - 512];
  }
  __syncthreads();
  if constexpr (PAIR) ptx::cluster_sync();
  pdl::sync_with_predecessor();

  if (warp < 4) {
    ptx::setmaxnreg_dec<40>();
    if (warp == 0 && ptx::elect_one()) {
      int stage = 0;
      uint32_t phase = 0;
      for (int item = first_item; item < total_items; item += item_stride) {
        const int tn = item % n_tiles, tm = (item / n_tiles) * (PAIR ? 2 : 1) + int(rank);
        int cb = 0, cy0 = 0, cx0 = 0;
        if (p.mode == 1) {
          cb = tm / (p.tiles_y * p.tiles_x);
          const int r = tm - cb * (p.tiles_y * p.tiles_x);
          cy0 = (r / p.tiles_x) * p.tile_h;
          cx0 = (r % p.tiles_x) * p.tile_w;
        }
        for (int kb = 0; kb < p.num_kb; ++kb) {
          ptx::mbar_wait(ptx::smem_u32(&empty_bar[stage]), phase ^ 1);
          const uint32_t fb = ptx::smem_u32(&full_bar[stage]);
          ptx::mbar_arrive_expect_tx(fb, C::kStageA + C::kStageB);
          const uint32_t sa = ptx::smem_u32(smem_a + stage * C::kStageA);
          const uint32_t sb = ptx::smem_u32(smem_b + stage * C::kStageB);
          int ka, kt = 0;
          if (p.mode == 1) {
            const int tap = kb / p.cin_blocks, cblk = kb - tap * p.cin_blocks;
            const int dy = tap / 3, dx = tap - dy * 3;
            ptx::tma_load_4d(sa, &tmap_a, fb, cblk * BLOCK_K, cx0 + dx - 1, cy0 + dy - 1, cb);
            ka = cblk * BLOCK_K;
            kt = tap;
          } else {
            ptx::tma_load_2d(sa, &tmap_a, fb, kb * BLOCK_K, tm * BLOCK_M);
            ka = kb * BLOCK_K;
          }
          if constexpr (PAIR) {
            constexpr int kHalf = BLOCK_N / 2;
            ptx::tma_load_3d_mc(sb + rank * (kHalf * BLOCK_K * 2), &tmap_b, fb, ka, kt, tn * BLOCK_N + int(rank) * kHalf, 0x3);
          } else {
            ptx::tma_load_3d(sb, &tmap_b, fb, ka, kt, tn * BLOCK_N);
          }
          if (++stage == C::kStages) { stage = 0; phase ^= 1; }
        }
      }
    }
  } else {
    ptx::setmaxnreg_inc<232>();
    const int wg = (threadIdx.x >> 7) - 1;
    const int wq = warp & 3;
    const int q = lane & 3;
    const uint32_t flags = p.flags & EpiMask<EPI>::value;
    constexpr int kNB = BLOCK_N / 8;
    float acc[BLOCK_N / 2];
    int stage = 0;
    uint32_t phase = 0;
    uint32_t out_chunk = 0;
    auto release = [&](int s) {
      if (lane == 0) {
        if constexpr (PAIR) {
          ptx::mbar_arrive_cluster(ptx::smem_u32(&empty_bar[s]), 0);
          ptx::mbar_arrive_cluster(ptx::smem_u32(&empty_bar[s]), 1);
        } else {
          ptx::mbar_arrive(ptx::smem_u32(&empty_bar[s]));
        }
      }
    };
    const bool conv_issuer = EPI == EPI_CONV && (threadIdx.x & 127) == 0;
    const bool conv_two = EPI == EPI_CONV && (flags & (F_OUT2_RELU | F_ADD1)) != 0;
    const bool conv_add = EPI == EPI_CONV && (flags & (F_ADD0 | F_ADD1)) != 0;
    uint32_t add_phase = 0;
    auto conv_box = [&](int tm, int& bx, int& by, int& bb) {
      bb = tm / (p.tiles_y * p.tiles_x);
      const int r = tm - bb * (p.tiles_y * p.tiles_x);
      bx = (r % p.tiles_x) * p.tile_w + (64 * wg) % p.tile_w;
      by = (r / p.tiles_x) * p.tile_h + (64 * wg) / p.tile_w;
    };
    auto out_buf = [&](int i) { return ptx::smem_u32(smem_o + (wg * 2 + i) * C::kOutBuf); };
    auto issue_addends = [&](int tm, int ch) {
      int bx, by, bb;
      conv_box(tm, bx, by, bb);
      const uint32_t b0 = conv_two ? out_buf(0) : out_buf(out_chunk & 1);
      if (conv_two) ptx::bulk_wait_group_read<0>();
      else ptx::bulk_wait_group_read<1>();
      const uint32_t bar = ptx::smem_u32(&add_bar[wg]);
      ptx::mbar_arrive_expect_tx(bar, uint32_t(C::kOutBuf) * (((flags & F_ADD0) ? 1u : 0u) + ((flags & F_ADD1) ? 1u : 0u)));
      if (flags & F_ADD0) ptx::tma_load_4d(b0, &cm->add0, bar, ch, bx, by, bb);
      if (flags & F_ADD1) ptx::tma_load_4d(out_buf(1), &cm->add1, bar, ch, bx, by, bb);
    };
    for (int item = first_item; item < total_items; item += item_stride) {
      const int tn = item % n_tiles, tm = (item / n_tiles) * (PAIR ? 2 : 1) + int(rank);
      if constexpr (EPI == EPI_CONV) {
        if (conv_add && conv_issuer) issue_addends(tm, tn * BLOCK_N);
      }
      int prev = -1;
      for (int kb = 0; kb < p.num_kb; ++kb) {
        ptx::mbar_wait(ptx::smem_u32(&full_bar[stage]), phase);
        const uint64_t da = ptx::desc_kmajor_sw128(ptx::smem_u32(smem_a + stage * C::kStageA + wg * 64 * 128));
        const uint64_t db = ptx::desc_kmajor_sw128(ptx::smem_u32(smem_b + stage * C::kStageB));
        ptx::wgmma_fence();
#pragma unroll
        for (int k = 0; k < BLOCK_K / WGMMA_K; ++k) {
          if constexpr (BLOCK_N == 256) ptx::wgmma_m64n256k16_ss(acc, da + uint64_t(2 * k), db + uint64_t(2 * k), (kb | k) != 0 ? 1u : 0u);
          else if constexpr (BLOCK_N == 128) ptx::wgmma_m64n128k16_ss(acc, da + uint64_t(2 * k), db + uint64_t(2 * k), (kb | k) != 0 ? 1u : 0u);
          else ptx::wgmma_m64n64k16_ss(acc, da + uint64_t(2 * k), db + uint64_t(2 * k), (kb | k) != 0 ? 1u : 0u);
        }
        ptx::wgmma_commit();
        ptx::wgmma_wait<1>();
        if (prev >= 0) release(prev);
        prev = stage;
        if (++stage == C::kStages) { stage = 0; phase ^= 1; }
      }
      ptx::wgmma_wait<0>();
      ptx::reg_fence(acc);
      release(prev);

      bool valid[2];
      long long row_off[2];
      int tok[2] = {0, 0};
      long long pix[2] = {0, 0};
      int ct_b[2] = {0, 0}, ct_iy[2] = {0, 0}, ct_ix[2] = {0, 0};
#pragma unroll
      for (int h = 0; h < 2; ++h) {
        const int row_in_tile = wg * 64 + wq * 16 + (lane >> 2) + 8 * h;
        if (p.mode == 1) {
          const int cb = tm / (p.tiles_y * p.tiles_x);
          const int r = tm - cb * (p.tiles_y * p.tiles_x);
          const int y = (r / p.tiles_x) * p.tile_h + row_in_tile / p.tile_w;
          const int x = (r % p.tiles_x) * p.tile_w + row_in_tile % p.tile_w;
          valid[h] = (tm < m_tiles) && (y < p.cH) && (x < p.cW);
          pix[h] = (long long)(cb * p.cH + y) * p.cW + x;
          row_off[h] = pix[h] * p.ldo;
        } else {
          const int row = tm * BLOCK_M + row_in_tile;
          valid[h] = row < p.M;
          row_off[h] = (long long)row * p.ldo;
          if (flags & F_ROPE) tok[h] = row % p.tokens_per_img;
          if (flags & F_CONVT) {
            ct_b[h] = row / (p.th_in * p.tw_in);
            const int r = row - ct_b[h] * (p.th_in * p.tw_in);
            ct_iy[h] = r / p.tw_in;
            ct_ix[h] = r - ct_iy[h] * p.tw_in;
          }
        }
      }
      if (flags & (F_BIAS | F_GELU)) {
#pragma unroll
        for (int j = 0; j < kNB; ++j) {
          const int c = tn * BLOCK_N + 8 * j + 2 * q;
          float2 b = make_float2(0.f, 0.f);
          if ((flags & F_BIAS) && c < p.N) {
            if (flags & F_CONVT) b = make_float2(__ldg(p.bias + c % p.tCout), __ldg(p.bias + (c + 1) % p.tCout));
            else b = __ldg(reinterpret_cast<const float2*>(p.bias + c));
          }
#pragma unroll
          for (int h = 0; h < 2; ++h) {
            float& v0 = acc[4 * j + 2 * h];
            float& v1 = acc[4 * j + 2 * h + 1];
            v0 += b.x;
            v1 += b.y;
            if (flags & F_GELU) { v0 = gelu_erf(v0); v1 = gelu_erf(v1); }
          }
        }
      }
      if (flags & F_ROPE) {
#pragma unroll
        for (int cb = 0; cb < BLOCK_N / 32; ++cb) {
          const int col0 = tn * BLOCK_N + cb * 32;
          if (col0 >= p.rope_cols) continue;
#pragma unroll
          for (int h = 0; h < 2; ++h) {
            const int pos = ((col0 & 63) < 32) ? (tok[h] / p.grid_w) : (tok[h] % p.grid_w);
#pragma unroll
            for (int jj = 0; jj < 2; ++jj) {
              const int k = 8 * jj + 2 * q;
              const float2 cs = __ldg(reinterpret_cast<const float2*>(p.rope_cos + pos * 16 + k));
              const float2 sn = __ldg(reinterpret_cast<const float2*>(p.rope_sin + pos * 16 + k));
              const float cc[2] = {cs.x, cs.y}, ss[2] = {sn.x, sn.y};
#pragma unroll
              for (int e = 0; e < 2; ++e) {
                float& u = acc[(4 * cb + jj) * 4 + 2 * h + e];
                float& w = acc[(4 * cb + jj + 2) * 4 + 2 * h + e];
                const float u0 = u, w0 = w;
                u = u0 * cc[e] - w0 * ss[e];
                w = w0 * cc[e] + u0 * ss[e];
              }
            }
          }
        }
      }
      if constexpr (EPI == EPI_CONV) {
        int bx, by, bb;
        conv_box(tm, bx, by, bb);
        const uint32_t sw = lane >> 2;
#pragma unroll
        for (int c = 0; c < BLOCK_N / 64; ++c) {
          const uint32_t b0 = conv_two ? out_buf(0) : out_buf(out_chunk & 1), b1 = out_buf(1);
          if (conv_add) {
            ptx::mbar_wait(ptx::smem_u32(&add_bar[wg]), add_phase);
            add_phase ^= 1;
          } else if (conv_two) {
            if (conv_issuer) ptx::bulk_wait_group_read<0>();
            ptx::named_bar_sync(1 + wg, 128);
          }
#pragma unroll
          for (int j = 0; j < 8; ++j)
#pragma unroll
            for (int h = 0; h < 2; ++h) {
              const uint32_t off = (wq * 16 + (lane >> 2) + 8 * h) * 128 + ((j ^ sw) << 4) + q * 4;
              float v0 = acc[4 * (c * 8 + j) + 2 * h], v1 = acc[4 * (c * 8 + j) + 2 * h + 1];
              if (flags & F_ADD0) {
                const float2 a = bf16x2_to_float2(ptx::ld_shared_b32(b0 + off));
                v0 += a.x; v1 += a.y;
              }
              if (flags & F_ADD1) {
                const float2 a = bf16x2_to_float2(ptx::ld_shared_b32(b1 + off));
                v0 += a.x; v1 += a.y;
              }
              if (flags & F_RELU) { v0 = fmaxf(v0, 0.f); v1 = fmaxf(v1, 0.f); }
              ptx::st_shared_b32(b0 + off, pack_bf16x2(v0, v1));
              if (flags & F_OUT2_RELU) ptx::st_shared_b32(b1 + off, pack_bf16x2(fmaxf(v0, 0.f), fmaxf(v1, 0.f)));
            }
          ptx::fence_proxy_async();
          if (!conv_add && !conv_two && conv_issuer) ptx::bulk_wait_group_read<0>();
          ptx::named_bar_sync(1 + wg, 128);
          const int ch = tn * BLOCK_N + c * 64;
          if (conv_issuer) {
            ptx::tma_store_4d(&tmap_o, b0, ch, bx, by, bb);
            if (flags & F_OUT2_RELU) ptx::tma_store_4d(&cm->out2, b1, ch, bx, by, bb);
            ptx::bulk_commit_group();
          }
          ++out_chunk;
          if (conv_add && conv_issuer && c + 1 < BLOCK_N / 64) issue_addends(tm, ch + 64);
        }
        continue;
      }
      if constexpr (TMA_STORE) {
        constexpr bool kF32 = (EPI == EPI_RESID);
        constexpr int kChunkCols = kF32 ? 32 : 64;
        constexpr int kChunkNB = kChunkCols / 8;
        const bool issuer = (threadIdx.x & 127) == 0;
        const uint32_t sw = lane >> 2;
#pragma unroll
        for (int c = 0; c < BLOCK_N / kChunkCols; ++c) {
          const uint32_t buf = ptx::smem_u32(smem_o + (wg * 2 + (out_chunk & 1)) * C::kOutBuf);
#pragma unroll
          for (int j = 0; j < kChunkNB; ++j)
#pragma unroll
            for (int h = 0; h < 2; ++h) {
              const uint32_t row = wq * 16 + (lane >> 2) + 8 * h;
              float v0 = acc[4 * (c * kChunkNB + j) + 2 * h], v1 = acc[4 * (c * kChunkNB + j) + 2 * h + 1];
              if (flags & F_RELU) { v0 = fmaxf(v0, 0.f); v1 = fmaxf(v1, 0.f); }
              if constexpr (kF32) {
                ptx::st_shared_v2_f32(buf + row * 128 + (((2 * j + (q >> 1)) ^ sw) << 4) + (q & 1) * 8, v0, v1);
              } else {
                ptx::st_shared_b32(buf + row * 128 + ((j ^ sw) << 4) + q * 4, pack_bf16x2(v0, v1));
              }
            }
          ptx::fence_proxy_async();
          if (issuer) ptx::bulk_wait_group_read<0>();
          ptx::named_bar_sync(1 + wg, 128);
          if (issuer) {
            const int c0 = tn * BLOCK_N + c * kChunkCols, r0 = tm * BLOCK_M + wg * 64;
            if constexpr (kF32) ptx::tma_reduce_add_2d(&tmap_o, buf, c0, r0);
            else ptx::tma_store_2d(&tmap_o, buf, c0, r0);
            ptx::bulk_commit_group();
          }
          ++out_chunk;
        }
        continue;
      }
      if (flags & F_HEAD_FINAL) {
        float head_acc[2][4] = {{0.f, 0.f, 0.f, 0.f}, {0.f, 0.f, 0.f, 0.f}};
#pragma unroll
        for (int j = 0; j < kNB; ++j)
#pragma unroll
          for (int h = 0; h < 2; ++h)
#pragma unroll
            for (int e = 0; e < 2; ++e) {
              const float r = fmaxf(acc[4 * j + 2 * h + e], 0.f);
              const int c = 8 * j + 2 * q + e;
#pragma unroll
              for (int o = 0; o < 4; ++o) head_acc[h][o] += r * s_w4[o * 128 + c];
            }
#pragma unroll
        for (int h = 0; h < 2; ++h)
#pragma unroll
          for (int o = 0; o < 4; ++o) {
            head_acc[h][o] += __shfl_xor_sync(0xffffffffu, head_acc[h][o], 1);
            head_acc[h][o] += __shfl_xor_sync(0xffffffffu, head_acc[h][o], 2);
          }
#pragma unroll
        for (int h = 0; h < 2; ++h) {
          if (!valid[h] || q != 0) continue;
          postprocess_pixel(head_acc[h][0] + s_w4[512 + 0], head_acc[h][1] + s_w4[512 + 1], head_acc[h][2] + s_w4[512 + 2],
                            [&] { return head_acc[h][3] + s_w4[512 + 3]; }, p.pts3d, p.conf, pix[h], p.depth_mode, p.conf_mode,
                            p.conf_min, p.conf_max);
        }
        continue;
      }
#pragma unroll
      for (int h = 0; h < 2; ++h) {
        if (!valid[h]) continue;
#pragma unroll
        for (int j = 0; j < kNB; ++j) {
          const int col = tn * BLOCK_N + 8 * j + 2 * q;
          if (col >= p.N) continue;
          float v0 = acc[4 * j + 2 * h], v1 = acc[4 * j + 2 * h + 1];
          long long off;
          if (flags & F_CONVT) {
            const int kk = col / p.tCout, co = col - kk * p.tCout;
            const int ky = kk / p.tk, kx = kk - ky * p.tk;
            off = ((long long)(ct_b[h] * p.th_in * p.tk + ct_iy[h] * p.tk + ky) * (p.tw_in * p.tk) + ct_ix[h] * p.tk + kx) * p.tCout + co;
          } else {
            off = row_off[h] + col;
          }
          if (flags & F_ADD0) {
            const float2 a = bf16x2_to_float2(__ldg(reinterpret_cast<const unsigned int*>(reinterpret_cast<const __nv_bfloat16*>(p.add0) + off)));
            v0 += a.x; v1 += a.y;
          }
          if (flags & F_ADD1) {
            const float2 a = bf16x2_to_float2(__ldg(reinterpret_cast<const unsigned int*>(reinterpret_cast<const __nv_bfloat16*>(p.add1) + off)));
            v0 += a.x; v1 += a.y;
          }
          if (flags & F_RELU) { v0 = fmaxf(v0, 0.f); v1 = fmaxf(v1, 0.f); }
          if (flags & (F_OUT_F32 | F_RESID_INPLACE)) {
            float2* o = reinterpret_cast<float2*>(reinterpret_cast<float*>(p.out) + off);
            if (flags & F_RESID_INPLACE) {
              const float2 r = *o;
              v0 += r.x; v1 += r.y;
            }
            *o = make_float2(v0, v1);
            if (flags & F_OUT2_BF16) *reinterpret_cast<uint32_t*>(reinterpret_cast<__nv_bfloat16*>(p.out2) + off) = pack_bf16x2(v0, v1);
          } else {
            *reinterpret_cast<uint32_t*>(reinterpret_cast<__nv_bfloat16*>(p.out) + off) = pack_bf16x2(v0, v1);
            if (flags & F_OUT2_RELU)
              *reinterpret_cast<uint32_t*>(reinterpret_cast<__nv_bfloat16*>(p.out2) + off) = pack_bf16x2(fmaxf(v0, 0.f), fmaxf(v1, 0.f));
          }
        }
      }
    }
    if constexpr (TMA_STORE) {
      if ((threadIdx.x & 127) == 0) ptx::bulk_wait_group<0>();
    }
  }
  if constexpr (PAIR) ptx::cluster_sync();
}

template <int BLOCK_N, int EPI, bool PAIR, bool TMA_STORE>
__global__ void __launch_bounds__(kNumThreads, 1)
gemm_kernel(const __grid_constant__ CUtensorMap tmap_a, const __grid_constant__ CUtensorMap tmap_b,
            const __grid_constant__ CUtensorMap tmap_o, const Params p) {
  gemm_body<BLOCK_N, EPI, PAIR, TMA_STORE>(tmap_a, tmap_b, tmap_o, nullptr, p);
}

template <int BLOCK_N, bool PAIR>
__global__ void __launch_bounds__(kNumThreads, 1)
conv_kernel(const __grid_constant__ CUtensorMap tmap_a, const __grid_constant__ CUtensorMap tmap_b,
            const __grid_constant__ CUtensorMap tmap_o, const __grid_constant__ ConvMaps cm, const Params p) {
  gemm_body<BLOCK_N, EPI_CONV, PAIR, true>(tmap_a, tmap_b, tmap_o, &cm, p);
}

}
}
```

### dust3r_b200/csrc/sm90_ptx.cuh

```cuda
#pragma once
#include <cuda.h>
#include <cuda_runtime.h>
#include <cuda_bf16.h>
#include <cstdint>

namespace d3r {
namespace ptx {

__device__ __forceinline__ uint32_t smem_u32(const void* p) { return static_cast<uint32_t>(__cvta_generic_to_shared(p)); }

__device__ __forceinline__ bool elect_one() {
  uint32_t pred = 0;
  asm volatile(
      "{\n"
      ".reg .b32 %%rx;\n"
      ".reg .pred %%px;\n"
      "elect.sync %%rx|%%px, %1;\n"
      "@%%px mov.s32 %0, 1;\n"
      "}\n"
      : "+r"(pred)
      : "r"(0xffffffffu));
  return pred != 0;
}

__device__ __forceinline__ void mbar_init(uint32_t bar, uint32_t count) {
  asm volatile("mbarrier.init.shared::cta.b64 [%0], %1;" ::"r"(bar), "r"(count));
}
__device__ __forceinline__ void fence_barrier_init() { asm volatile("fence.mbarrier_init.release.cluster;" ::: "memory"); }
__device__ __forceinline__ void fence_proxy_async() { asm volatile("fence.proxy.async.shared::cta;" ::: "memory"); }

__device__ __forceinline__ void mbar_arrive_expect_tx(uint32_t bar, uint32_t bytes) {
  asm volatile("mbarrier.arrive.expect_tx.shared::cta.b64 _, [%0], %1;" ::"r"(bar), "r"(bytes) : "memory");
}
__device__ __forceinline__ void mbar_arrive(uint32_t bar) {
  asm volatile("mbarrier.arrive.shared::cta.b64 _, [%0];" ::"r"(bar) : "memory");
}
__device__ __forceinline__ bool mbar_try_wait(uint32_t bar, uint32_t parity) {
  uint32_t done;
  asm volatile(
      "{\n"
      ".reg .pred p;\n"
      "mbarrier.try_wait.parity.shared::cta.b64 p, [%1], %2;\n"
      "selp.u32 %0, 1, 0, p;\n"
      "}\n"
      : "=r"(done)
      : "r"(bar), "r"(parity)
      : "memory");
  return done != 0;
}
__device__ __forceinline__ void mbar_wait(uint32_t bar, uint32_t parity) {
  while (!mbar_try_wait(bar, parity)) {
  }
}
__device__ __forceinline__ void mbar_wait_bounded(uint32_t bar, uint32_t parity) {
  uint32_t spins = 0;
  bool done;
  do {
    done = mbar_try_wait(bar, parity);
    if (!done && ++spins > (1u << 22)) __trap();
  } while (!done);
}

__device__ __forceinline__ void bulk_g2s(uint32_t dst, const void* src, uint32_t bytes, uint32_t bar) {
  asm volatile("cp.async.bulk.shared::cluster.global.mbarrier::complete_tx::bytes [%0], [%1], %2, [%3];"
               ::"r"(dst), "l"(src), "r"(bytes), "r"(bar) : "memory");
}
__device__ __forceinline__ uint64_t policy_evict_first() {
  uint64_t pol;
  asm volatile("createpolicy.fractional.L2::evict_first.b64 %0, 1.0;" : "=l"(pol));
  return pol;
}
__device__ __forceinline__ void bulk_g2s_hint(uint32_t dst, const void* src, uint32_t bytes, uint32_t bar, uint64_t pol) {
  asm volatile("cp.async.bulk.shared::cluster.global.mbarrier::complete_tx::bytes.L2::cache_hint [%0], [%1], %2, [%3], %4;"
               ::"r"(dst), "l"(src), "r"(bytes), "r"(bar), "l"(pol) : "memory");
}

__device__ __forceinline__ void prefetch_tmap(const void* tmap) {
  asm volatile("prefetch.tensormap [%0];" ::"l"(reinterpret_cast<uint64_t>(tmap)) : "memory");
}
__device__ __forceinline__ void tma_load_2d(uint32_t dst, const void* tmap, uint32_t bar, int c0, int c1) {
  asm volatile(
      "cp.async.bulk.tensor.2d.shared::cluster.global.mbarrier::complete_tx::bytes [%0], [%1, {%3, %4}], [%2];"
      ::"r"(dst), "l"(reinterpret_cast<uint64_t>(tmap)), "r"(bar), "r"(c0), "r"(c1)
      : "memory");
}
__device__ __forceinline__ void tma_load_3d(uint32_t dst, const void* tmap, uint32_t bar, int c0, int c1, int c2) {
  asm volatile(
      "cp.async.bulk.tensor.3d.shared::cluster.global.mbarrier::complete_tx::bytes [%0], [%1, {%3, %4, %5}], [%2];"
      ::"r"(dst), "l"(reinterpret_cast<uint64_t>(tmap)), "r"(bar), "r"(c0), "r"(c1), "r"(c2)
      : "memory");
}
__device__ __forceinline__ void tma_load_4d(uint32_t dst, const void* tmap, uint32_t bar, int c0, int c1, int c2, int c3) {
  asm volatile(
      "cp.async.bulk.tensor.4d.shared::cluster.global.mbarrier::complete_tx::bytes [%0], [%1, {%3, %4, %5, %6}], [%2];"
      ::"r"(dst), "l"(reinterpret_cast<uint64_t>(tmap)), "r"(bar), "r"(c0), "r"(c1), "r"(c2), "r"(c3)
      : "memory");
}
__device__ __forceinline__ void tma_load_3d_mc(uint32_t dst, const void* tmap, uint32_t bar, int c0, int c1, int c2, uint16_t mask) {
  asm volatile(
      "cp.async.bulk.tensor.3d.shared::cluster.global.mbarrier::complete_tx::bytes.multicast::cluster [%0], [%1, {%3, %4, %5}], [%2], %6;"
      ::"r"(dst), "l"(reinterpret_cast<uint64_t>(tmap)), "r"(bar), "r"(c0), "r"(c1), "r"(c2), "h"(mask)
      : "memory");
}

__device__ __forceinline__ void tma_store_2d(const void* tmap, uint32_t src, int c0, int c1) {
  asm volatile("cp.async.bulk.tensor.2d.global.shared::cta.tile.bulk_group [%0, {%2, %3}], [%1];"
               ::"l"(reinterpret_cast<uint64_t>(tmap)), "r"(src), "r"(c0), "r"(c1) : "memory");
}
__device__ __forceinline__ void tma_store_4d(const void* tmap, uint32_t src, int c0, int c1, int c2, int c3) {
  asm volatile("cp.async.bulk.tensor.4d.global.shared::cta.tile.bulk_group [%0, {%2, %3, %4, %5}], [%1];"
               ::"l"(reinterpret_cast<uint64_t>(tmap)), "r"(src), "r"(c0), "r"(c1), "r"(c2), "r"(c3) : "memory");
}
__device__ __forceinline__ void tma_reduce_add_2d(const void* tmap, uint32_t src, int c0, int c1) {
  asm volatile("cp.reduce.async.bulk.tensor.2d.global.shared::cta.add.tile.bulk_group [%0, {%2, %3}], [%1];"
               ::"l"(reinterpret_cast<uint64_t>(tmap)), "r"(src), "r"(c0), "r"(c1) : "memory");
}
__device__ __forceinline__ void bulk_commit_group() { asm volatile("cp.async.bulk.commit_group;" ::: "memory"); }
template <int N> __device__ __forceinline__ void bulk_wait_group_read() { asm volatile("cp.async.bulk.wait_group.read %0;" ::"n"(N) : "memory"); }
template <int N> __device__ __forceinline__ void bulk_wait_group() { asm volatile("cp.async.bulk.wait_group %0;" ::"n"(N) : "memory"); }
__device__ __forceinline__ void st_shared_b32(uint32_t addr, uint32_t v) { asm volatile("st.shared.b32 [%0], %1;" ::"r"(addr), "r"(v) : "memory"); }
__device__ __forceinline__ uint32_t ld_shared_b32(uint32_t addr) {
  uint32_t v;
  asm volatile("ld.shared.b32 %0, [%1];" : "=r"(v) : "r"(addr) : "memory");
  return v;
}
__device__ __forceinline__ void st_shared_v2_f32(uint32_t addr, float a, float b) {
  asm volatile("st.shared.v2.f32 [%0], {%1, %2};" ::"r"(addr), "f"(a), "f"(b) : "memory");
}
__device__ __forceinline__ void named_bar_sync(uint32_t id, uint32_t count) { asm volatile("bar.sync %0, %1;" ::"r"(id), "r"(count) : "memory"); }

__device__ __forceinline__ uint32_t cluster_ctarank() {
  uint32_t r;
  asm volatile("mov.u32 %0, %%cluster_ctarank;" : "=r"(r));
  return r;
}
__device__ __forceinline__ void cluster_sync() {
  asm volatile("barrier.cluster.arrive.release.aligned;\nbarrier.cluster.wait.acquire.aligned;" ::: "memory");
}
__device__ __forceinline__ void mbar_arrive_cluster(uint32_t bar, uint32_t rank) {
  asm volatile(
      "{\n"
      ".reg .b32 raddr;\n"
      "mapa.shared::cluster.u32 raddr, %0, %1;\n"
      "mbarrier.arrive.shared::cluster.b64 _, [raddr];\n"
      "}\n" ::"r"(bar), "r"(rank) : "memory");
}

__device__ __forceinline__ float ex2_approx(float x) { float y; asm("ex2.approx.ftz.f32 %0, %1;" : "=f"(y) : "f"(x)); return y; }
__device__ __forceinline__ float rcp_approx(float x) { float y; asm("rcp.approx.ftz.f32 %0, %1;" : "=f"(y) : "f"(x)); return y; }
__device__ __forceinline__ float rsqrt_approx(float x) { float y; asm("rsqrt.approx.ftz.f32 %0, %1;" : "=f"(y) : "f"(x)); return y; }
__device__ __forceinline__ float sqrt_approx(float x) { float y; asm("sqrt.approx.ftz.f32 %0, %1;" : "=f"(y) : "f"(x)); return y; }

template <int N> __device__ __forceinline__ void setmaxnreg_dec() { asm volatile("setmaxnreg.dec.sync.aligned.u32 %0;" ::"n"(N)); }
template <int N> __device__ __forceinline__ void setmaxnreg_inc() { asm volatile("setmaxnreg.inc.sync.aligned.u32 %0;" ::"n"(N)); }

__device__ __forceinline__ void wgmma_fence() { asm volatile("wgmma.fence.sync.aligned;" ::: "memory"); }
__device__ __forceinline__ void wgmma_commit() { asm volatile("wgmma.commit_group.sync.aligned;" ::: "memory"); }
template <int N> __device__ __forceinline__ void wgmma_wait() { asm volatile("wgmma.wait_group.sync.aligned %0;" ::"n"(N) : "memory"); }
template <int N> __device__ __forceinline__ void reg_fence(float (&d)[N]) {
#pragma unroll
  for (int i = 0; i < N; ++i) asm volatile("" : "+f"(d[i])::"memory");
}

__device__ __forceinline__ uint64_t desc_sw128(uint32_t smem_addr, uint32_t lbo_bytes) {
  uint64_t d = 0;
  d |= uint64_t((smem_addr & 0x3FFFF) >> 4);
  d |= uint64_t(lbo_bytes >> 4) << 16;
  d |= uint64_t(1024 >> 4) << 32;
  d |= uint64_t(1) << 62;
  return d;
}
__device__ __forceinline__ uint64_t desc_kmajor_sw128(uint32_t smem_addr) { return desc_sw128(smem_addr, 16); }
__device__ __forceinline__ uint64_t desc_mnmajor_sw128(uint32_t smem_addr) { return desc_sw128(smem_addr, 1024); }

__device__ __forceinline__ void wgmma_m64n64k16_ss(float* d, uint64_t desc_a, uint64_t desc_b, uint32_t accumulate) {
  asm volatile(
      "{\n"
      ".reg .pred p;\n"
      "setp.ne.b32 p, %34, 0;\n"
      "wgmma.mma_async.sync.aligned.m64n64k16.f32.bf16.bf16 "
      "{%0, %1, %2, %3, %4, %5, %6, %7, %8, %9, %10, %11, %12, %13, %14, %15, %16, %17, %18, %19, %20, %21, %22, %23, %24, %25, %26, %27, %28, %29, %30, %31}, %32, %33, p, 1, 1, 0, 0;\n"
      "}\n"
      : "+f"(d[0]), "+f"(d[1]), "+f"(d[2]), "+f"(d[3]), "+f"(d[4]), "+f"(d[5]), "+f"(d[6]), "+f"(d[7]), "+f"(d[8]), "+f"(d[9]), "+f"(d[10]), "+f"(d[11]), "+f"(d[12]), "+f"(d[13]), "+f"(d[14]), "+f"(d[15]), "+f"(d[16]), "+f"(d[17]), "+f"(d[18]), "+f"(d[19]), "+f"(d[20]), "+f"(d[21]), "+f"(d[22]), "+f"(d[23]), "+f"(d[24]), "+f"(d[25]), "+f"(d[26]), "+f"(d[27]), "+f"(d[28]), "+f"(d[29]), "+f"(d[30]), "+f"(d[31])
      : "l"(desc_a), "l"(desc_b), "r"(accumulate));
}
__device__ __forceinline__ void wgmma_m64n128k16_ss(float* d, uint64_t desc_a, uint64_t desc_b, uint32_t accumulate) {
  asm volatile(
      "{\n"
      ".reg .pred p;\n"
      "setp.ne.b32 p, %66, 0;\n"
      "wgmma.mma_async.sync.aligned.m64n128k16.f32.bf16.bf16 "
      "{%0, %1, %2, %3, %4, %5, %6, %7, %8, %9, %10, %11, %12, %13, %14, %15, %16, %17, %18, %19, %20, %21, %22, %23, %24, %25, %26, %27, %28, %29, %30, %31, %32, %33, %34, %35, %36, %37, %38, %39, %40, %41, %42, %43, %44, %45, %46, %47, %48, %49, %50, %51, %52, %53, %54, %55, %56, %57, %58, %59, %60, %61, %62, %63}, %64, %65, p, 1, 1, 0, 0;\n"
      "}\n"
      : "+f"(d[0]), "+f"(d[1]), "+f"(d[2]), "+f"(d[3]), "+f"(d[4]), "+f"(d[5]), "+f"(d[6]), "+f"(d[7]), "+f"(d[8]), "+f"(d[9]), "+f"(d[10]), "+f"(d[11]), "+f"(d[12]), "+f"(d[13]), "+f"(d[14]), "+f"(d[15]), "+f"(d[16]), "+f"(d[17]), "+f"(d[18]), "+f"(d[19]), "+f"(d[20]), "+f"(d[21]), "+f"(d[22]), "+f"(d[23]), "+f"(d[24]), "+f"(d[25]), "+f"(d[26]), "+f"(d[27]), "+f"(d[28]), "+f"(d[29]), "+f"(d[30]), "+f"(d[31]), "+f"(d[32]), "+f"(d[33]), "+f"(d[34]), "+f"(d[35]), "+f"(d[36]), "+f"(d[37]), "+f"(d[38]), "+f"(d[39]), "+f"(d[40]), "+f"(d[41]), "+f"(d[42]), "+f"(d[43]), "+f"(d[44]), "+f"(d[45]), "+f"(d[46]), "+f"(d[47]), "+f"(d[48]), "+f"(d[49]), "+f"(d[50]), "+f"(d[51]), "+f"(d[52]), "+f"(d[53]), "+f"(d[54]), "+f"(d[55]), "+f"(d[56]), "+f"(d[57]), "+f"(d[58]), "+f"(d[59]), "+f"(d[60]), "+f"(d[61]), "+f"(d[62]), "+f"(d[63])
      : "l"(desc_a), "l"(desc_b), "r"(accumulate));
}
__device__ __forceinline__ void wgmma_m64n256k16_ss(float* d, uint64_t desc_a, uint64_t desc_b, uint32_t accumulate) {
  asm volatile(
      "{\n"
      ".reg .pred p;\n"
      "setp.ne.b32 p, %130, 0;\n"
      "wgmma.mma_async.sync.aligned.m64n256k16.f32.bf16.bf16 "
      "{%0, %1, %2, %3, %4, %5, %6, %7, %8, %9, %10, %11, %12, %13, %14, %15, %16, %17, %18, %19, %20, %21, %22, %23, %24, %25, %26, %27, %28, %29, %30, %31, %32, %33, %34, %35, %36, %37, %38, %39, %40, %41, %42, %43, %44, %45, %46, %47, %48, %49, %50, %51, %52, %53, %54, %55, %56, %57, %58, %59, %60, %61, %62, %63, %64, %65, %66, %67, %68, %69, %70, %71, %72, %73, %74, %75, %76, %77, %78, %79, %80, %81, %82, %83, %84, %85, %86, %87, %88, %89, %90, %91, %92, %93, %94, %95, %96, %97, %98, %99, %100, %101, %102, %103, %104, %105, %106, %107, %108, %109, %110, %111, %112, %113, %114, %115, %116, %117, %118, %119, %120, %121, %122, %123, %124, %125, %126, %127}, %128, %129, p, 1, 1, 0, 0;\n"
      "}\n"
      : "+f"(d[0]), "+f"(d[1]), "+f"(d[2]), "+f"(d[3]), "+f"(d[4]), "+f"(d[5]), "+f"(d[6]), "+f"(d[7]), "+f"(d[8]), "+f"(d[9]), "+f"(d[10]), "+f"(d[11]), "+f"(d[12]), "+f"(d[13]), "+f"(d[14]), "+f"(d[15]), "+f"(d[16]), "+f"(d[17]), "+f"(d[18]), "+f"(d[19]), "+f"(d[20]), "+f"(d[21]), "+f"(d[22]), "+f"(d[23]), "+f"(d[24]), "+f"(d[25]), "+f"(d[26]), "+f"(d[27]), "+f"(d[28]), "+f"(d[29]), "+f"(d[30]), "+f"(d[31]), "+f"(d[32]), "+f"(d[33]), "+f"(d[34]), "+f"(d[35]), "+f"(d[36]), "+f"(d[37]), "+f"(d[38]), "+f"(d[39]), "+f"(d[40]), "+f"(d[41]), "+f"(d[42]), "+f"(d[43]), "+f"(d[44]), "+f"(d[45]), "+f"(d[46]), "+f"(d[47]), "+f"(d[48]), "+f"(d[49]), "+f"(d[50]), "+f"(d[51]), "+f"(d[52]), "+f"(d[53]), "+f"(d[54]), "+f"(d[55]), "+f"(d[56]), "+f"(d[57]), "+f"(d[58]), "+f"(d[59]), "+f"(d[60]), "+f"(d[61]), "+f"(d[62]), "+f"(d[63]), "+f"(d[64]), "+f"(d[65]), "+f"(d[66]), "+f"(d[67]), "+f"(d[68]), "+f"(d[69]), "+f"(d[70]), "+f"(d[71]), "+f"(d[72]), "+f"(d[73]), "+f"(d[74]), "+f"(d[75]), "+f"(d[76]), "+f"(d[77]), "+f"(d[78]), "+f"(d[79]), "+f"(d[80]), "+f"(d[81]), "+f"(d[82]), "+f"(d[83]), "+f"(d[84]), "+f"(d[85]), "+f"(d[86]), "+f"(d[87]), "+f"(d[88]), "+f"(d[89]), "+f"(d[90]), "+f"(d[91]), "+f"(d[92]), "+f"(d[93]), "+f"(d[94]), "+f"(d[95]), "+f"(d[96]), "+f"(d[97]), "+f"(d[98]), "+f"(d[99]), "+f"(d[100]), "+f"(d[101]), "+f"(d[102]), "+f"(d[103]), "+f"(d[104]), "+f"(d[105]), "+f"(d[106]), "+f"(d[107]), "+f"(d[108]), "+f"(d[109]), "+f"(d[110]), "+f"(d[111]), "+f"(d[112]), "+f"(d[113]), "+f"(d[114]), "+f"(d[115]), "+f"(d[116]), "+f"(d[117]), "+f"(d[118]), "+f"(d[119]), "+f"(d[120]), "+f"(d[121]), "+f"(d[122]), "+f"(d[123]), "+f"(d[124]), "+f"(d[125]), "+f"(d[126]), "+f"(d[127])
      : "l"(desc_a), "l"(desc_b), "r"(accumulate));
}
__device__ __forceinline__ void wgmma_m64n64k16_rs_tb(float* d, const uint32_t* a, uint64_t desc_b, uint32_t accumulate) {
  asm volatile(
      "{\n"
      ".reg .pred p;\n"
      "setp.ne.b32 p, %37, 0;\n"
      "wgmma.mma_async.sync.aligned.m64n64k16.f32.bf16.bf16 "
      "{%0, %1, %2, %3, %4, %5, %6, %7, %8, %9, %10, %11, %12, %13, %14, %15, %16, %17, %18, %19, %20, %21, %22, %23, %24, %25, %26, %27, %28, %29, %30, %31}, {%32, %33, %34, %35}, %36, p, 1, 1, 1;\n"
      "}\n"
      : "+f"(d[0]), "+f"(d[1]), "+f"(d[2]), "+f"(d[3]), "+f"(d[4]), "+f"(d[5]), "+f"(d[6]), "+f"(d[7]), "+f"(d[8]), "+f"(d[9]), "+f"(d[10]), "+f"(d[11]), "+f"(d[12]), "+f"(d[13]), "+f"(d[14]), "+f"(d[15]), "+f"(d[16]), "+f"(d[17]), "+f"(d[18]), "+f"(d[19]), "+f"(d[20]), "+f"(d[21]), "+f"(d[22]), "+f"(d[23]), "+f"(d[24]), "+f"(d[25]), "+f"(d[26]), "+f"(d[27]), "+f"(d[28]), "+f"(d[29]), "+f"(d[30]), "+f"(d[31])
      : "r"(a[0]), "r"(a[1]), "r"(a[2]), "r"(a[3]), "l"(desc_b), "r"(accumulate));
}
__device__ __forceinline__ void wgmma_m64n64k16_ss_tb(float* d, uint64_t desc_a, uint64_t desc_b, uint32_t accumulate) {
  asm volatile(
      "{\n"
      ".reg .pred p;\n"
      "setp.ne.b32 p, %34, 0;\n"
      "wgmma.mma_async.sync.aligned.m64n64k16.f32.bf16.bf16 "
      "{%0, %1, %2, %3, %4, %5, %6, %7, %8, %9, %10, %11, %12, %13, %14, %15, %16, %17, %18, %19, %20, %21, %22, %23, %24, %25, %26, %27, %28, %29, %30, %31}, %32, %33, p, 1, 1, 0, 1;\n"
      "}\n"
      : "+f"(d[0]), "+f"(d[1]), "+f"(d[2]), "+f"(d[3]), "+f"(d[4]), "+f"(d[5]), "+f"(d[6]), "+f"(d[7]), "+f"(d[8]), "+f"(d[9]), "+f"(d[10]), "+f"(d[11]), "+f"(d[12]), "+f"(d[13]), "+f"(d[14]), "+f"(d[15]), "+f"(d[16]), "+f"(d[17]), "+f"(d[18]), "+f"(d[19]), "+f"(d[20]), "+f"(d[21]), "+f"(d[22]), "+f"(d[23]), "+f"(d[24]), "+f"(d[25]), "+f"(d[26]), "+f"(d[27]), "+f"(d[28]), "+f"(d[29]), "+f"(d[30]), "+f"(d[31])
      : "l"(desc_a), "l"(desc_b), "r"(accumulate));
}

}
}
```

### include/dust3r_b200.h

```cpp
#ifndef DUST3R_B200_H_
#define DUST3R_B200_H_

#include <stddef.h>
#include <stdint.h>

#ifdef __cplusplus
extern "C" {
#endif

#define D3R_OK 0
#define D3R_ERR_INVALID (-1)
#define D3R_ERR_CUDA (-2)
#define D3R_ERR_UNSUPPORTED_DEVICE (-3)

const char* d3r_last_error(void);
int d3r_abi_version(void);
int d3r_check_device(void);

long long d3r_launch_count(void);
void d3r_launch_count_reset(void);
void d3r_prof_enable(int on);
int d3r_prof_report(char* buf, int cap);
int d3r_prof_dump(char* buf, int cap);


typedef struct d3r_align_desc {
  int32_t n_imgs;
  int32_t n_edges;
  int32_t n_entries;
  int32_t n_chunks;
  int32_t max_deg;
  int32_t max_chunks;
  int32_t chunk_px;
  int32_t dist_l2;
  int32_t norm_pw_scale;
  int32_t tied_focal;
  int32_t eval_only;
  float base_scale;
  float pw_break;
  float focal_break;
  float adam_eps;
  float beta1, beta2;

  const int32_t* img_hw;
  const int64_t* img_pix_off;
  const int32_t* img_ent_ptr;
  const int32_t* img_chunk_ptr;
  const int32_t* chunk_img;
  const int32_t* ent_edge;
  const int64_t* ent_obs_off;
  const float*   ent_coef;
  const int32_t* edge_ent;
  const void* obs;

  float* logd;
  float* logd_m;
  float* logd_v;
  float* small;
  float* small_m;
  float* small_v;
  const uint8_t* small_trainable;

  float* workspace;
  const float* sched;
  float* loss_out;
  int32_t* counters;

  int32_t stream_kernel;
  int32_t stream_grid;
  int32_t stream_ppt;
  int32_t stream_window;
  int32_t n_items;
  int32_t reserved0;
  const void* items;
  const int32_t* warp_item_ptr;
  const void* items_rev;
  const int32_t* warp_item_ptr_rev;
} d3r_align_desc;

typedef struct d3r_align_item {
  int32_t img, slot0, nslots, npx;
  int32_t e0, deg, W, u0;
  int32_t v0;
  float inv_w;
  int64_t pix0;
  int64_t obs0;
  int32_t slab_units;
  int32_t reserved;
} d3r_align_item;

int d3r_sizeof_align_desc(void);
int d3r_sizeof_align_item(void);
int d3r_align_chunk_pixels(void);
int64_t d3r_align_workspace_floats(int32_t n_imgs, int32_t n_edges);
int d3r_align_prepare(const d3r_align_desc* desc, void* stream);
int d3r_align_run(const d3r_align_desc* desc, int32_t it_begin, int32_t it_end, void* stream);
int d3r_align_pixel_pass(const d3r_align_desc* desc, int32_t it, void* stream);
int d3r_align_small_step(const d3r_align_desc* desc, int32_t it, void* stream);
int d3r_align_reduce_block(int32_t n_imgs, int32_t n_edges, int64_t* offset_floats, int64_t* n_words);
int d3r_align_grad_pixel_pass(const d3r_align_desc* desc, float* logd_grad, void* stream);
int d3r_align_grad_small_step(const d3r_align_desc* desc, float* small_grad, float* entry_loss, void* stream);
int d3r_align_loss_grad(const d3r_align_desc* desc, float* logd_grad, float* small_grad, float* entry_loss, void* stream);
int d3r_align_overflow_flag(const d3r_align_desc* desc, int32_t* host_out, void* stream);
int d3r_align_pts3d(const d3r_align_desc* desc, float* out_dev, void* stream);
int d3r_align_set_debug(void* dev_buf);

#define D3R_CONF_ID 0
#define D3R_CONF_LOG 1
#define D3R_CONF_SQRT 2
#define D3R_CONF_M1 3
typedef struct d3r_pack_entry {
  const float* pts;
  const float* conf;
  int64_t obs_off;
  int32_t area;
  float coef;
} d3r_pack_entry;
int d3r_sizeof_pack_entry(void);
int d3r_align_stream_slots_per_item(void);
int d3r_align_stream_warps_per_cta(void);
int d3r_align_stream_max_window(void);
int d3r_align_pack_entries(const d3r_pack_entry* table_dev, int32_t n_entries, int32_t max_area, int32_t conf_mode,
                           int32_t stream_layout, void* obs_dev, void* stream);


#define D3R_F_BIAS          (1u << 0)
#define D3R_F_GELU          (1u << 1)
#define D3R_F_RELU          (1u << 2)
#define D3R_F_OUT_F32       (1u << 3)
#define D3R_F_RESID_INPLACE (1u << 4)
#define D3R_F_ADD0          (1u << 5)
#define D3R_F_ADD1          (1u << 6)
#define D3R_F_OUT2_RELU     (1u << 7)
#define D3R_F_ROPE          (1u << 8)
#define D3R_F_OUT2_BF16     (1u << 11)

int d3r_gemm_bf16(const void* A_dev, const void* B_dev, void* out_dev, const float* bias_dev, const void* add0_dev,
                  void* out2_dev, int32_t M, int32_t N, int32_t K, int64_t ldo, uint32_t flags,
                  const float* rope_cos_dev, const float* rope_sin_dev, int32_t rope_cols, int32_t tokens_per_img,
                  int32_t grid_w, void* stream);

int d3r_conv3x3_bf16(const void* x_nhwc_dev, const void* w_packed_dev, void* out_dev, const float* bias_dev,
                     const void* add0_dev, const void* add1_dev, void* out2_dev, int32_t B, int32_t H, int32_t W,
                     int32_t Cin, int32_t Cout, uint32_t flags, void* stream);

int d3r_attention_hd64(const void* q_dev, int64_t ldq, const void* k_dev, int64_t ldk, const void* v_dev, int64_t ldv,
                       void* out_dev, int64_t ldo, int32_t B, int32_t heads, int32_t Nq, int32_t Nk, float scale,
                       void* stream);

int d3r_conv_transpose_bf16(const void* x_nhwc_dev, const void* w_packed_dev, void* out_dev, const float* bias_dev, int32_t B,
                            int32_t h, int32_t w, int32_t Cin, int32_t Cout, int32_t k, void* stream);

int d3r_conv3x3_head_tail(const void* x_nhwc_dev, const void* w_packed_dev, const float* bias_dev, const float* w4_dev,
                          const float* b4_dev, float* pts3d_dev, float* conf_dev, int32_t B, int32_t H, int32_t W, int32_t depth_mode,
                          int32_t conf_mode, float conf_min, float conf_max, void* stream);

int d3r_layernorm_bf16(const float* x_dev, const float* g_dev, const float* b_dev, void* out_dev, int32_t M, int32_t C, float eps,
                       void* stream);

int d3r_upsample2x_bf16(const void* x_dev, void* out_dev, int32_t B, int32_t H, int32_t W, int32_t C, int32_t Ho, int32_t Wo,
                        void* stream);

int d3r_im2col_3x3_s2_bf16(const void* x_dev, void* out_dev, int32_t B, int32_t H, int32_t W, int32_t C, void* stream);

int d3r_patch_im2col16(const float* img_dev, void* out_dev, int32_t B, int32_t H, int32_t W, void* stream);

int d3r_linear_head_postprocess(const float* feat_dev, float* pts3d_dev, float* conf_dev, int32_t B, int32_t gh, int32_t gw,
                                int32_t nch, int32_t depth_mode, int32_t conf_mode, float conf_min, float conf_max, void* stream);

void d3r_set_gemm_impl(int32_t impl);
void d3r_set_gemm_store(int32_t store);
void d3r_set_conv_store(int32_t store);

void d3r_set_attention_impl(int32_t impl);

int d3r_clean_pointcloud(int32_t n_imgs, const int32_t* hw_dev, const int64_t* off_dev, int32_t max_area, const float* pts3d_dev,
                         float* conf_dev, const float* depth_dev, const float* K_dev, const float* cams_dev, float tol,
                         float bad_conf, void* stream);
int d3r_procrustes_moments(int32_t n_problems, int32_t n_points, const float* x_dev, const float* y_dev, const float* w_dev,
                           double* out_dev, void* stream);
int d3r_weiszfeld_focal(int32_t n_maps, int32_t H, int32_t W, const float* pts3d_dev, const float* pp_dev, int32_t steps,
                        float* focal_dev, void* stream);
int d3r_nearest_neighbours(int32_t n_queries, int32_t n_points, const float* queries_dev, const float* points_dev, int32_t* nn_dev,
                           void* stream);
int d3r_image_resize_crop_normalize(const uint8_t* src_dev, int32_t H0, int32_t W0, int32_t H1, int32_t W1,
                                    const int32_t* xbounds_dev, const int32_t* xcoefs_dev, int32_t kx,
                                    const int32_t* ybounds_dev, const int32_t* ycoefs_dev, int32_t ky, int32_t row0, int32_t rows,
                                    int32_t crop_x0, int32_t crop_y0, int32_t H2, int32_t W2, const float* lut_dev, uint8_t* tmp_dev,
                                    float* out_dev, void* stream);
typedef struct d3r_view_desc {
  const uint8_t* src;
  const float* depth;
  int32_t src_pitch, depth_pitch;
  int32_t H0, W0;
  int32_t H1, W1;
  int32_t crop_x0, crop_y0;
  int32_t H2, W2;
  int32_t row0, rows;
  int32_t transpose, reserved;
  const int32_t* xbounds;
  const int32_t* xcoefs;
  const int32_t* ybounds;
  const int32_t* ycoefs;
  float fu, fv, cu, cv;
  float pose[12];
  uint8_t* tmp;
  float* img;
  float* depthmap;
  float* pts3d;
  uint8_t* valid;
  int64_t blocks[3];
} d3r_view_desc;

int32_t d3r_sizeof_view_desc(void);
int d3r_prepare_views(int32_t n_views, const d3r_view_desc* desc, d3r_view_desc* desc_dev, const float* lut_dev, void* stream);
typedef struct d3r_jpeg_huff {
  int32_t maxcode[18];
  int32_t valoff[18];
  uint16_t look[512];
  uint8_t val[256];
} d3r_jpeg_huff;

typedef struct d3r_jpeg_desc {
  int32_t width, height;
  int32_t n_comp;
  int32_t restart_interval;
  int32_t orientation;
  int32_t reserved;
  int64_t scan_begin;
  int32_t h_samp[3], v_samp[3];
  int32_t dc_table[3], ac_table[3];
  uint16_t quant[3][64];
  d3r_jpeg_huff huff[8];
} d3r_jpeg_desc;

#define D3R_JPEG_BAD_CODE 1
#define D3R_JPEG_SHORT 2
#define D3R_JPEG_BAD_RESTART 4
#define D3R_JPEG_MARKER_COUNT 8
#define D3R_JPEG_RANGE 16

int32_t d3r_sizeof_jpeg_desc(void);
int64_t d3r_jpeg_decode_workspace_bytes(const d3r_jpeg_desc* desc, int64_t n_bytes);
int d3r_jpeg_decode(const d3r_jpeg_desc* desc, const uint8_t* data_dev, int64_t n_bytes, uint8_t* out_dev, int32_t* status_dev,
                    void* workspace_dev, int64_t workspace_bytes, void* stream);

typedef struct d3r_png_desc {
  int32_t width, height;
  int32_t color_type;
  int32_t orientation;
  int32_t palette_len;
  int32_t reserved;
  int64_t idat_bytes;
  uint8_t palette[256][3];
} d3r_png_desc;

#define D3R_PNG_BAD_CODE 1
#define D3R_PNG_FAR 2
#define D3R_PNG_SHORT 4
#define D3R_PNG_ADLER 8
#define D3R_PNG_FILTER 16
#define D3R_PNG_PALETTE 32

int32_t d3r_sizeof_png_desc(void);
int64_t d3r_png_decode_workspace_bytes(const d3r_png_desc* desc, int64_t n_bytes);
int d3r_png_decode(const d3r_png_desc* desc, const uint8_t* zdata_dev, int64_t n_bytes, uint8_t* out_dev, int32_t* status_dev,
                   void* workspace_dev, int64_t workspace_bytes, void* stream);

int64_t d3r_segment_sky_workspace_bytes(int32_t n_imgs, int64_t total_px);
int d3r_segment_sky(int32_t n_imgs, const int32_t* hw_dev, const int64_t* off_dev, int32_t max_area, int64_t total_px,
                    const uint8_t* rgb_dev, uint8_t* sky_out_dev, void* workspace_dev, int64_t workspace_bytes, void* stream);

int64_t d3r_nanmedian_workspace_bytes(int32_t n_seg);
int d3r_segmented_nanmedian(int32_t n_seg, int64_t seg_len, const float* vals_dev, float* out_dev, void* workspace_dev,
                            int64_t workspace_bytes, void* stream);
int64_t d3r_criterion_workspace_bytes(int32_t B, int64_t n1, int64_t n2, int32_t flags);
int d3r_criterion(int32_t B, int64_t n1, int64_t n2, int32_t flags, int32_t reduction, float dist_clip, float alpha,
                  const float* T_dev, const float* gt1_dev, const float* gt2_dev, const uint8_t* valid1_dev, const uint8_t* valid2_dev,
                  const float* pr1_dev, const float* pr2_dev, const float* conf1_dev, const float* conf2_dev, float* out_dev,
                  float* pix1_dev, float* pix2_dev, uint8_t* mask1_dev, uint8_t* mask2_dev, void* workspace_dev,
                  int64_t workspace_bytes, void* stream);


int64_t d3r_pnp_ransac_workspace_bytes(int32_t max_iters);
int d3r_pnp_ransac(int32_t n, const float* pts2d_dev, const float* pts3d_dev, double fx, double fy, double cx, double cy,
                   double threshold, double confidence, int32_t max_iters, int64_t seed, void* workspace_dev, int64_t workspace_bytes,
                   int32_t* result_dev, double* pose_dev, uint8_t* mask_dev, void* stream);
int d3r_pnp_hypotheses(int32_t n, const float* pts2d_dev, const float* pts3d_dev, double fx, double fy, double cx, double cy,
                       double threshold, int64_t seed, int32_t h0, int32_t n_hyp, int32_t* idx_dev, double* pose_dev,
                       int32_t* counts_dev, void* stream);

typedef struct d3r_linear { const void* w; const float* b; } d3r_linear;
typedef struct d3r_norm { const float* g; const float* b; } d3r_norm;

typedef struct d3r_enc_block {
  d3r_norm norm1, norm2;
  d3r_linear qkv, proj, fc1, fc2;
} d3r_enc_block;

typedef struct d3r_dec_block {
  d3r_norm norm1, norm2, norm3, norm_y;
  d3r_linear qkv, proj;
  d3r_linear projq, projkv, cproj;
  d3r_linear fc1, fc2;
} d3r_dec_block;

typedef struct d3r_fusion {
  d3r_linear rcu1_conv1, rcu1_conv2, rcu2_conv1, rcu2_conv2;
  d3r_linear out_conv;
} d3r_fusion;

typedef struct d3r_dpt_head {
  d3r_linear act_conv[4];
  d3r_linear act0_up;
  d3r_linear act1_up;
  d3r_linear act3_down;
  d3r_linear layer_rn[4];
  d3r_fusion refine[4];
  d3r_linear head0;
  d3r_linear head2;
  const float* head4_w;
  const float* head4_b;
} d3r_dpt_head;

typedef struct d3r_model {
  int32_t enc_dim, enc_depth, enc_heads, dec_dim, dec_depth, dec_heads, mlp_ratio, patch;
  int32_t head_type;
  int32_t nch;
  int32_t depth_mode;
  int32_t conf_mode;
  float conf_min, conf_max, ln_eps;
  int32_t hooks[4];
  int32_t rope_max_pos;
  const float* rope_cos;
  const float* rope_sin;
  d3r_linear patch_embed;
  const d3r_enc_block* enc;
  d3r_norm enc_norm;
  d3r_linear decoder_embed;
  const d3r_dec_block* dec1;
  const d3r_dec_block* dec2;
  d3r_norm dec_norm;
  const d3r_dpt_head* dpt[2];
  d3r_linear lin_head[2];
} d3r_model;

int d3r_sizeof_model(void);

int64_t d3r_encode_workspace_bytes(const d3r_model* m, int32_t n, int32_t H, int32_t W);
int d3r_encode_images(const d3r_model* m, const float* imgs_dev, int32_t n, int32_t H, int32_t W, void* feat_dev,
                      void* workspace_dev, int64_t workspace_bytes, void* stream);
int64_t d3r_decode_workspace_bytes(const d3r_model* m, int32_t B, int32_t H1, int32_t W1, int32_t H2, int32_t W2);
int d3r_decode_pairs(const d3r_model* m, const void* feat1_dev, int32_t n1, int32_t H1, int32_t W1, const void* feat2_dev,
                     int32_t n2, int32_t H2, int32_t W2, const int32_t* idx1_host, const int32_t* idx2_host, int32_t B,
                     float* pts3d_1, float* conf_1, float* pts3d_2, float* conf_2, void* workspace_dev,
                     int64_t workspace_bytes, void* stream);

int d3r_forward_set_debug(int32_t stage_id, float* out_dev, int64_t capacity_floats);

#ifdef __cplusplus
}
#endif
#endif
```

Measured before the change: 233.2.

## Fuse residual GEMM with following LayerNorm via cluster-wide row statistics

Adds a clustered WGMMA kernel that computes the residual-add GEMM and then applies one or two LayerNorms in the epilogue. Each CTA in a cluster of 3 or 4 owns a 256-column slice, and per-row mean/M2 partials are exchanged through st.async to remote shared memory. The encoder and decoder call it for proj, cproj, fc2, patch embedding and decoder embedding, which removes the standalone layernorm launches and the extra fp32 reads of x. It also fuses the cross-branch norm_y LayerNorm into the other branch's fc2 using double-buffered ynorm buffers. The cost is a cluster barrier per tile, restriction to N of 768 or 1024, and fewer CTAs, since each M-tile is spread across a whole cluster.

New measurement: 236.3, median of 6. +1.3%, better.

```diff
diff --git a/dust3r_b200/_lib.py b/dust3r_b200/_lib.py
--- a/dust3r_b200/_lib.py
+++ b/dust3r_b200/_lib.py
@@ -101,6 +101,7 @@
     'd3r_align_stream_max_window': (i32, []),
     'd3r_align_pack_entries': (i32, [vp, i32, i32, i32, i32, vp, vp]),
     'd3r_gemm_bf16': (i32, [vp, vp, vp, vp, vp, vp, i32, i32, i32, i64, u32, vp, vp, i32, i32, i32, vp]),
+    'd3r_gemm_resid_ln': (i32, [vp, vp, vp, vp, i32, i32, i32, i32, vp, vp, vp, vp, vp, vp, f32, vp]),
     'd3r_conv3x3_bf16': (i32, [vp, vp, vp, vp, vp, vp, vp, i32, i32, i32, i32, i32, u32, vp]),
     'd3r_attention_hd64': (i32, [vp, i64, vp, i64, vp, i64, vp, i64, i32, i32, i32, i32, f32, vp]),
     'd3r_conv_transpose_bf16': (i32, [vp, vp, vp, vp, i32, i32, i32, i32, i32, i32, vp]),
diff --git a/dust3r_b200/csrc/c_api.cu b/dust3r_b200/csrc/c_api.cu
--- a/dust3r_b200/csrc/c_api.cu
+++ b/dust3r_b200/csrc/c_api.cu
@@ -29,7 +29,7 @@
                                   CUtensorMapL2promotion, CUtensorMapFloatOOBfill);
 
 int encode_tensor_map(CUtensorMap* m, const void* base, int rank, const cuuint64_t* dims, const cuuint64_t* strides_bytes,
-                      const cuuint32_t* box, const char* op, CUtensorMapDataType dtype) {
+                      const cuuint32_t* box, const char* op, CUtensorMapDataType dtype, CUtensorMapSwizzle swizzle) {
   static EncodeTiledFn fn = nullptr;
   static std::once_flag once;
   std::call_once(once, [] {
@@ -44,7 +44,7 @@
   }
   const cuuint32_t estr[5] = {1, 1, 1, 1, 1};
   CUresult r = fn(m, dtype, (cuuint32_t)rank, const_cast<void*>(base), dims, strides_bytes, box, estr,
-                  CU_TENSOR_MAP_INTERLEAVE_NONE, CU_TENSOR_MAP_SWIZZLE_128B, CU_TENSOR_MAP_L2_PROMOTION_L2_256B,
+                  CU_TENSOR_MAP_INTERLEAVE_NONE, swizzle, CU_TENSOR_MAP_L2_PROMOTION_L2_256B,
                   CU_TENSOR_MAP_FLOAT_OOB_FILL_NONE);
   if (r != CUDA_SUCCESS) {
     set_error("%s: cuTensorMapEncodeTiled failed with CUresult %d (rank %d, dims %llu,%llu)", op, (int)r, rank,
diff --git a/dust3r_b200/csrc/d3r_common.cuh b/dust3r_b200/csrc/d3r_common.cuh
--- a/dust3r_b200/csrc/d3r_common.cuh
+++ b/dust3r_b200/csrc/d3r_common.cuh
@@ -80,7 +80,8 @@
 int num_sms();
 
 int encode_tensor_map(CUtensorMap* m, const void* base, int rank, const cuuint64_t* dims, const cuuint64_t* strides_bytes,
-                      const cuuint32_t* box, const char* op, CUtensorMapDataType dtype = CU_TENSOR_MAP_DATA_TYPE_BFLOAT16);
+                      const cuuint32_t* box, const char* op, CUtensorMapDataType dtype = CU_TENSOR_MAP_DATA_TYPE_BFLOAT16,
+                      CUtensorMapSwizzle swizzle = CU_TENSOR_MAP_SWIZZLE_128B);
 
 inline bool first_launch_on_this_device(unsigned long long& mask) {
   int dev = 0;
diff --git a/dust3r_b200/csrc/forward.cu b/dust3r_b200/csrc/forward.cu
--- a/dust3r_b200/csrc/forward.cu
+++ b/dust3r_b200/csrc/forward.cu
@@ -70,6 +70,31 @@
   return gemm::conv3x3_bf16(x, w.w, B, H, W, Cin, Cout, p, c.st);
 }
 
+struct LnOut {
+  const d3r_norm* n;
+  __nv_bfloat16* out;
+};
+
+static int resid_ln(const Ctx& c, const void* A, long long lda, const d3r_linear& w, int M, int N, int K, float* x, bool resid,
+                    LnOut y0, LnOut y1 = {nullptr, nullptr}) {
+  if (gemm::resid_ln_supported(N, K) && !(resid && N == 1024 && K >= 4 * N)) {
+    Params p{};
+    p.M = M; p.N = N; p.K = K;
+    p.flags = (resid ? gemm::F_RESID_INPLACE : 0u) | (w.b ? gemm::F_BIAS : 0u);
+    p.out = x; p.bias = w.b;
+    p.ln_g[0] = y0.n->g; p.ln_b[0] = y0.n->b;
+    if (y1.out) { p.ln_g[1] = y1.n->g; p.ln_b[1] = y1.n->b; }
+    p.ln_outs = y1.out ? 2 : 1;
+    p.ln_eps = c.m->ln_eps;
+    void* const y[2] = {y0.out, y1.out};
+    return gemm::gemm_resid_ln(A, lda, w.w, p, y, c.st);
+  }
+  RC(linear(c, A, lda, w, M, N, K, x, resid ? gemm::F_RESID_INPLACE : gemm::F_OUT_F32));
+  RC(ew::layernorm(x, y0.n->g, y0.n->b, y0.out, nullptr, M, N, c.m->ln_eps, c.st));
+  if (y1.out) RC(ew::layernorm(x, y1.n->g, y1.n->b, y1.out, nullptr, M, N, c.m->ln_eps, c.st));
+  return D3R_OK;
+}
+
 static int run_encoder(const Ctx& c, Arena& ar, const float* imgs, int n_enc, int H, int W, __nv_bfloat16* eout) {
   const d3r_model& m = *c.m;
   const int E = m.enc_dim, M = n_enc * c.N, hid = E * m.mlp_ratio, pk = 3 * m.patch * m.patch;
@@ -79,47 +104,42 @@
   __nv_bfloat16* att = ar.arr<__nv_bfloat16>((size_t)M * E);
   __nv_bfloat16* hidb = ar.arr<__nv_bfloat16>((size_t)M * (hid > pk ? hid : pk));
   if (ar.dry) return D3R_OK;
+  auto next_ln = [&](int l) { return l < m.enc_depth ? LnOut{&m.enc[l].norm1, ln} : LnOut{&m.enc_norm, eout}; };
   RC(ew::patch_im2col16(imgs, hidb, n_enc, H, W, c.st));
-  RC(linear(c, hidb, pk, m.patch_embed, M, E, pk, x, gemm::F_OUT_F32));
+  RC(resid_ln(c, hidb, pk, m.patch_embed, M, E, pk, x, false, next_ln(0)));
   tap_f32(1, x, (size_t)M * E, c.st);
   const float scale = 1.0f / sqrtf(float(E / m.enc_heads));
   for (int l = 0; l < m.enc_depth; ++l) {
     const d3r_enc_block& b = m.enc[l];
-    RC(ew::layernorm(x, b.norm1.g, b.norm1.b, ln, nullptr, M, E, m.ln_eps, c.st));
     RC(linear(c, ln, E, b.qkv, M, 3 * E, E, qkv, gemm::F_ROPE, nullptr, nullptr, 2 * E));
     RC(attn::attention_hd64(qkv, 3 * E, qkv + E, 3 * E, qkv + 2 * E, 3 * E, att, E, n_enc, m.enc_heads, c.N, c.N, scale, c.st));
-    RC(linear(c, att, E, b.proj, M, E, E, x, gemm::F_RESID_INPLACE));
-    RC(ew::layernorm(x, b.norm2.g, b.norm2.b, ln, nullptr, M, E, m.ln_eps, c.st));
+    RC(resid_ln(c, att, E, b.proj, M, E, E, x, true, LnOut{&b.norm2, ln}));
     RC(linear(c, ln, E, b.fc1, M, hid, E, hidb, gemm::F_GELU));
-    RC(linear(c, hidb, hid, b.fc2, M, E, hid, x, gemm::F_RESID_INPLACE));
+    RC(resid_ln(c, hidb, hid, b.fc2, M, E, hid, x, true, next_ln(l + 1)));
     if (l == 0) tap_f32(2, x, (size_t)M * E, c.st);
   }
   tap_f32(3, x, (size_t)M * E, c.st);
-  RC(ew::layernorm(x, m.enc_norm.g, m.enc_norm.b, eout, nullptr, M, E, m.ln_eps, c.st));
   tap_bf16(4, eout, (size_t)M * E, c.st);
   return D3R_OK;
 }
 
 struct DecBufs {
-  __nv_bfloat16 *ln, *qkv, *att, *q, *kv, *hid;
+  __nv_bfloat16 *qkv, *att, *q, *kv, *hid;
 };
-static int dec_block(const Ctx& c, const Ctx& cy, const d3r_dec_block& b, float* x, const __nv_bfloat16* ynorm, const DecBufs& w,
-                     int B) {
+static int dec_block(const Ctx& c, const Ctx& cy, const d3r_dec_block& b, float* x, __nv_bfloat16* ln, const __nv_bfloat16* ynorm,
+                     const DecBufs& w, int B, LnOut nxt0, LnOut nxt1) {
   const d3r_model& m = *c.m;
   const int D = m.dec_dim, M = B * c.N, My = B * cy.N, hid = D * m.mlp_ratio;
   const float scale = 1.0f / sqrtf(float(D / m.dec_heads));
-  RC(ew::layernorm(x, b.norm1.g, b.norm1.b, w.ln, nullptr, M, D, m.ln_eps, c.st));
-  RC(linear(c, w.ln, D, b.qkv, M, 3 * D, D, w.qkv, gemm::F_ROPE, nullptr, nullptr, 2 * D));
+  RC(linear(c, ln, D, b.qkv, M, 3 * D, D, w.qkv, gemm::F_ROPE, nullptr, nullptr, 2 * D));
   RC(attn::attention_hd64(w.qkv, 3 * D, w.qkv + D, 3 * D, w.qkv + 2 * D, 3 * D, w.att, D, B, m.dec_heads, c.N, c.N, scale, c.st));
-  RC(linear(c, w.att, D, b.proj, M, D, D, x, gemm::F_RESID_INPLACE));
-  RC(ew::layernorm(x, b.norm2.g, b.norm2.b, w.ln, nullptr, M, D, m.ln_eps, c.st));
-  RC(linear(c, w.ln, D, b.projq, M, D, D, w.q, gemm::F_ROPE, nullptr, nullptr, D));
+  RC(resid_ln(c, w.att, D, b.proj, M, D, D, x, true, LnOut{&b.norm2, ln}));
+  RC(linear(c, ln, D, b.projq, M, D, D, w.q, gemm::F_ROPE, nullptr, nullptr, D));
   RC(linear(cy, ynorm, D, b.projkv, My, 2 * D, D, w.kv, gemm::F_ROPE, nullptr, nullptr, D));
   RC(attn::attention_hd64(w.q, D, w.kv, 2 * D, w.kv + D, 2 * D, w.att, D, B, m.dec_heads, c.N, cy.N, scale, c.st));
-  RC(linear(c, w.att, D, b.cproj, M, D, D, x, gemm::F_RESID_INPLACE));
-  RC(ew::layernorm(x, b.norm3.g, b.norm3.b, w.ln, nullptr, M, D, m.ln_eps, c.st));
-  RC(linear(c, w.ln, D, b.fc1, M, hid, D, w.hid, gemm::F_GELU));
-  RC(linear(c, w.hid, hid, b.fc2, M, D, hid, x, gemm::F_RESID_INPLACE));
+  RC(resid_ln(c, w.att, D, b.cproj, M, D, D, x, true, LnOut{&b.norm3, ln}));
+  RC(linear(c, ln, D, b.fc1, M, hid, D, w.hid, gemm::F_GELU));
+  RC(resid_ln(c, w.hid, hid, b.fc2, M, D, hid, x, true, nxt0, nxt1));
   return D3R_OK;
 }
 
@@ -214,9 +234,13 @@
   f[1] = ar.arr<bf>((size_t)Md[1] * E);
   int* maps = ar.arr<int>((size_t)2 * B);
   float* x[2] = {ar.arr<float>((size_t)Md[0] * D), ar.arr<float>((size_t)Md[1] * D)};
-  bf* yn[2] = {ar.arr<bf>((size_t)Md[1] * D), ar.arr<bf>((size_t)Md[0] * D)};
+  bf* yn[2][2];
+  for (int k = 0; k < 2; ++k) {
+    yn[0][k] = ar.arr<bf>((size_t)Md[1] * D);
+    yn[1][k] = ar.arr<bf>((size_t)Md[0] * D);
+  }
+  bf* ln[2] = {ar.arr<bf>((size_t)Md[0] * D), ar.arr<bf>((size_t)Md[1] * D)};
   DecBufs w;
-  w.ln = ar.arr<bf>((size_t)Mx * D);
   w.qkv = ar.arr<bf>((size_t)Mx * 3 * D);
   w.att = ar.arr<bf>((size_t)Mx * D);
   w.q = ar.arr<bf>((size_t)Mx * D);
@@ -252,14 +276,28 @@
     RC(ew::gather_images_bf16(enc[br], f[br], maps + br * B, B, cv[br].N, E, st));
   }
 
-  RC(linear(cv[0], f[0], E, m.decoder_embed, Md[0], D, E, x[0], gemm::F_OUT_F32));
-  RC(linear(cv[1], f[1], E, m.decoder_embed, Md[1], D, E, x[1], gemm::F_OUT_F32));
+  const d3r_dec_block* blk[2] = {m.dec1, m.dec2};
+  auto next_ln = [&](int br, int l, LnOut& a, LnOut& b) {
+    if (l < m.dec_depth) {
+      a = LnOut{&blk[br][l].norm1, ln[br]};
+      b = LnOut{&blk[1 - br][l].norm_y, yn[1 - br][l & 1]};
+    } else {
+      a = LnOut{&m.dec_norm, hook[br][2]};
+      b = LnOut{nullptr, nullptr};
+    }
+  };
+  for (int br = 0; br < 2; ++br) {
+    LnOut a, b;
+    next_ln(br, 0, a, b);
+    RC(resid_ln(cv[br], f[br], E, m.decoder_embed, Md[br], D, E, x[br], false, a, b));
+  }
   tap_f32(5, x[0], (size_t)Md[0] * D, st);
   for (int l = 0; l < m.dec_depth; ++l) {
-    RC(ew::layernorm(x[1], m.dec1[l].norm_y.g, m.dec1[l].norm_y.b, yn[0], nullptr, Md[1], D, m.ln_eps, st));
-    RC(ew::layernorm(x[0], m.dec2[l].norm_y.g, m.dec2[l].norm_y.b, yn[1], nullptr, Md[0], D, m.ln_eps, st));
-    RC(dec_block(cv[0], cv[1], m.dec1[l], x[0], yn[0], w, B));
-    RC(dec_block(cv[1], cv[0], m.dec2[l], x[1], yn[1], w, B));
+    for (int br = 0; br < 2; ++br) {
+      LnOut a, b;
+      next_ln(br, l + 1, a, b);
+      RC(dec_block(cv[br], cv[1 - br], blk[br][l], x[br], ln[br], yn[br][l & 1], w, B, a, b));
+    }
     if (l == 0) { tap_f32(6, x[0], (size_t)Md[0] * D, st); tap_f32(7, x[1], (size_t)Md[1] * D, st); }
     for (int k = 1; k <= 2; ++k) {
       if (m.head_type == 1 && l + 1 == m.hooks[k]) {
@@ -270,8 +308,6 @@
   }
   tap_f32(8, x[0], (size_t)Md[0] * D, st);
   tap_f32(9, x[1], (size_t)Md[1] * D, st);
-  RC(ew::layernorm(x[0], m.dec_norm.g, m.dec_norm.b, hook[0][2], nullptr, Md[0], D, m.ln_eps, st));
-  RC(ew::layernorm(x[1], m.dec_norm.g, m.dec_norm.b, hook[1][2], nullptr, Md[1], D, m.ln_eps, st));
 
   float* outs[2][2] = {{pts1, conf1}, {pts2, conf2}};
   if (m.head_type == 0) {
diff --git a/dust3r_b200/csrc/gemm_host.cu b/dust3r_b200/csrc/gemm_host.cu
--- a/dust3r_b200/csrc/gemm_host.cu
+++ b/dust3r_b200/csrc/gemm_host.cu
@@ -20,6 +20,8 @@
 
 static int g_store = 1;
 static int g_conv_store = 1;
+
+static bool aligned16(const void* ptr) { return (reinterpret_cast<uintptr_t>(ptr) & 15) == 0; }
 
 static int grid_for(bool pair, int m_tiles, int n_tiles) {
   if (pair) {
@@ -148,6 +150,103 @@
   return dispatch(bn, ta, tb, staged ? &to : nullptr, p, (p.M + BLOCK_M - 1) / BLOCK_M, st);
 }
 
+bool resid_ln_supported(int N, int K) { return (N == 768 || N == 1024) && K % 8 == 0 && (K + BLOCK_K - 1) / BLOCK_K >= 3; }
+
+template <int RC>
+static int launch_resid_ln(const CUtensorMap& ta, const CUtensorMap& tb, const CUtensorMap& y0, const CUtensorMap& y1, const CUtensorMap& tx,
+                           const Params& p, int m_tiles, cudaStream_t st) {
+  constexpr int kSmem = Cfg<256, true, true>::kSmemBytes;
+  static unsigned long long attr_devices = 0;
+  static int max_clusters[64] = {};
+  int dev = 0;
+  D3R_CUDA(cudaGetDevice(&dev));
+  if (first_launch_on_this_device(attr_devices)) {
+    D3R_CUDA(cudaFuncSetAttribute(resid_ln_kernel<RC>, cudaFuncAttributeMaxDynamicSharedMemorySize, kSmem));
+    cudaLaunchConfig_t cfg = {};
+    cfg.gridDim = dim3(RC * (num_sms() / RC));
+    cfg.blockDim = dim3(kNumThreads);
+    cfg.dynamicSmemBytes = kSmem;
+    cudaLaunchAttribute at;
+    at.id = cudaLaunchAttributeClusterDimension;
+    at.val.clusterDim.x = RC;
+    at.val.clusterDim.y = 1;
+    at.val.clusterDim.z = 1;
+    cfg.attrs = &at;
+    cfg.numAttrs = 1;
+    int n = 0;
+    D3R_CUDA(cudaOccupancyMaxActiveClusters(&n, resid_ln_kernel<RC>, &cfg));
+    if (n <= 0) {
+      set_error("gemm_resid_ln: no cluster of %d CTAs fits on the device", RC);
+      return D3R_ERR_CUDA;
+    }
+    max_clusters[dev & 63] = n;
+  }
+  const int clusters = m_tiles < max_clusters[dev & 63] ? m_tiles : max_clusters[dev & 63];
+  char detail[96];
+  const unsigned gemm_flags = (unsigned)(p.flags | ((p.flags & F_RESID_INPLACE) ? 0u : F_OUT_F32));
+  snprintf(detail, sizeof(detail), "M=%d N=%d K=%d flags=0x%x mode=0 epi=%d", p.M, p.N, p.K, gemm_flags, EPI_RESID_LN);
+  const double mn = double(p.M) * double(p.N);
+  prof::Scope scope("gemm_wgmma_resid_ln", st, 2.0 * mn * double(p.K), mn * ((p.flags & F_RESID_INPLACE) ? 8.0 : 4.0) + mn * 2.0 * p.ln_outs, 1,
+                    detail);
+  D3R_CUDA(pdl::launch_clustered(resid_ln_kernel<RC>, dim3(clusters * RC), dim3(kNumThreads), size_t(kSmem), st, RC, ta, tb, y0, y1, tx, p));
+  D3R_LAUNCH_CHECK();
+  return D3R_OK;
+}
+
+int gemm_resid_ln(const void* A, long long lda, const void* B, Params p, void* const y[2], cudaStream_t st) {
+  D3R_CHECK_ARG(A && B && p.out && y[0], "gemm_resid_ln: null buffer");
+  D3R_CHECK_ARG(p.M > 0 && p.K > 0, "gemm_resid_ln: bad shape %d %d %d", p.M, p.N, p.K);
+  D3R_CHECK_ARG(resid_ln_supported(p.N, p.K), "gemm_resid_ln: N=%d must be 768 or 1024 and K=%d a multiple of 8 of at least 129", p.N,
+                p.K);
+  D3R_CHECK_ARG(lda % 8 == 0 && lda >= p.K, "gemm_resid_ln: lda=%lld", lda);
+  D3R_CHECK_ARG(p.ln_outs == 1 || p.ln_outs == 2, "gemm_resid_ln: %d LayerNorm outputs", p.ln_outs);
+  D3R_CHECK_ARG((p.flags & ~EpiMask<EPI_RESID_LN>::value) == 0, "gemm_resid_ln: flags 0x%x", (unsigned)p.flags);
+  D3R_CHECK_ARG(!(p.flags & F_BIAS) || p.bias, "gemm_resid_ln: F_BIAS without bias");
+  for (int o = 0; o < p.ln_outs; ++o)
+    D3R_CHECK_ARG(y[o] && p.ln_g[o] && p.ln_b[o] && aligned16(y[o]) && (reinterpret_cast<uintptr_t>(p.ln_g[o]) & 7) == 0 &&
+                      (reinterpret_cast<uintptr_t>(p.ln_b[o]) & 7) == 0,
+                  "gemm_resid_ln: LayerNorm output %d: null or misaligned buffer", o);
+  D3R_CHECK_ARG(aligned16(A) && aligned16(B) && aligned16(p.out) && (!p.bias || (reinterpret_cast<uintptr_t>(p.bias) & 7) == 0),
+                "gemm_resid_ln: operands and x must be 16-byte aligned");
+  p.mode = 0;
+  p.ldo = p.N;
+  p.num_kb = (p.K + BLOCK_K - 1) / BLOCK_K;
+  const int rc_n = p.N / 256;
+  CUtensorMap ta, tb, ty[2], tx;
+  {
+    cuuint64_t dims[2] = {(cuuint64_t)p.K, (cuuint64_t)p.M};
+    cuuint64_t str[1] = {(cuuint64_t)lda * 2};
+    cuuint32_t box[2] = {(cuuint32_t)BLOCK_K, (cuuint32_t)(rc_n == 4 ? 32 : 64)};
+    int rc = encode_tensor_map(&ta, A, 2, dims, str, box, "gemm_resid_ln");
+    if (rc) return rc;
+  }
+  {
+    cuuint64_t dims[3] = {(cuuint64_t)p.K, 1, (cuuint64_t)p.N};
+    cuuint64_t str[2] = {(cuuint64_t)p.K * 2, (cuuint64_t)p.K * 2};
+    cuuint32_t box[3] = {(cuuint32_t)BLOCK_K, 1, 256};
+    int rc = encode_tensor_map(&tb, B, 3, dims, str, box, "gemm_resid_ln");
+    if (rc) return rc;
+  }
+  for (int o = 0; o < 2; ++o) {
+    cuuint64_t dims[2] = {(cuuint64_t)p.N, (cuuint64_t)p.M};
+    cuuint64_t str[1] = {(cuuint64_t)p.N * 2};
+    cuuint32_t box[2] = {32, 64};
+    int rc = encode_tensor_map(&ty[o], y[o < p.ln_outs ? o : 0], 2, dims, str, box, "gemm_resid_ln output", CU_TENSOR_MAP_DATA_TYPE_BFLOAT16,
+                               CU_TENSOR_MAP_SWIZZLE_64B);
+    if (rc) return rc;
+  }
+  {
+    cuuint64_t dims[2] = {(cuuint64_t)p.N, (cuuint64_t)p.M};
+    cuuint64_t str[1] = {(cuuint64_t)p.N * 4};
+    cuuint32_t box[2] = {32, 64};
+    int rc = encode_tensor_map(&tx, p.out, 2, dims, str, box, "gemm_resid_ln x", CU_TENSOR_MAP_DATA_TYPE_FLOAT32);
+    if (rc) return rc;
+  }
+  const int m_tiles = (p.M + BLOCK_M - 1) / BLOCK_M;
+  return rc_n == 4 ? launch_resid_ln<4>(ta, tb, ty[0], ty[1], tx, p, m_tiles, st)
+                   : launch_resid_ln<3>(ta, tb, ty[0], ty[1], tx, p, m_tiles, st);
+}
+
 static int make_tmap_conv_io(CUtensorMap* m, const void* base, int B, int H, int W, int C, int tile_w, const char* op) {
   const int bw = tile_w < 64 ? tile_w : 64;
   cuuint64_t dims[4] = {(cuuint64_t)C, (cuuint64_t)W, (cuuint64_t)H, (cuuint64_t)B};
@@ -155,8 +254,6 @@
   cuuint32_t box[4] = {64, (cuuint32_t)bw, (cuuint32_t)(64 / bw), 1};
   return encode_tensor_map(m, base, 4, dims, str, box, op);
 }
-
-static bool aligned16(const void* ptr) { return (reinterpret_cast<uintptr_t>(ptr) & 15) == 0; }
 
 int conv3x3_bf16(const void* x_nhwc, const void* w_packed, int B, int H, int W, int Cin, int Cout, Params p, cudaStream_t st) {
   D3R_CHECK_ARG(x_nhwc && w_packed, "conv3x3: null operand");
@@ -266,6 +363,20 @@
   return gemm::gemm_bf16(A, K, B, p, (cudaStream_t)stream);
 }
 
+extern "C" int d3r_gemm_resid_ln(const void* A, const void* B, float* x, const float* bias, int32_t M, int32_t N, int32_t K, int32_t resid,
+                                 const float* g0, const float* b0, void* y0, const float* g1, const float* b1, void* y1, float eps,
+                                 void* stream) {
+  gemm::Params p{};
+  p.M = M; p.N = N; p.K = K;
+  p.flags = (bias ? gemm::F_BIAS : 0u) | (resid ? gemm::F_RESID_INPLACE : 0u);
+  p.out = x; p.bias = bias;
+  p.ln_g[0] = g0; p.ln_b[0] = b0; p.ln_g[1] = g1; p.ln_b[1] = b1;
+  p.ln_outs = y1 ? 2 : 1;
+  p.ln_eps = eps;
+  void* const y[2] = {y0, y1};
+  return gemm::gemm_resid_ln(A, K, B, p, y, (cudaStream_t)stream);
+}
+
 extern "C" int d3r_conv3x3_bf16(const void* x_nhwc, const void* w_packed, void* out, const float* bias, const void* add0,
                                 const void* add1, void* out2, int32_t B, int32_t H, int32_t W, int32_t Cin, int32_t Cout,
                                 uint32_t flags, void* stream) {
diff --git a/dust3r_b200/csrc/gemm_host.h b/dust3r_b200/csrc/gemm_host.h
--- a/dust3r_b200/csrc/gemm_host.h
+++ b/dust3r_b200/csrc/gemm_host.h
@@ -4,6 +4,8 @@
 namespace d3r {
 namespace gemm {
 int gemm_bf16(const void* A, long long lda, const void* B, Params p, cudaStream_t st);
+bool resid_ln_supported(int N, int K);
+int gemm_resid_ln(const void* A, long long lda, const void* B, Params p, void* const y[2], cudaStream_t st);
 int conv3x3_bf16(const void* x_nhwc, const void* w_packed, int B, int H, int W, int Cin, int Cout, Params p, cudaStream_t st);
 int conv_transpose_bf16(const void* x_nhwc, const void* w_packed, void* out, const float* bias, int B, int h, int w, int Cin, int Cout,
                         int k, cudaStream_t st);
diff --git a/dust3r_b200/csrc/gemm_wgmma.cuh b/dust3r_b200/csrc/gemm_wgmma.cuh
--- a/dust3r_b200/csrc/gemm_wgmma.cuh
+++ b/dust3r_b200/csrc/gemm_wgmma.cuh
@@ -50,14 +50,19 @@
   int depth_mode;
   int conf_mode;
   float conf_min, conf_max;
+  const float* ln_g[2];
+  const float* ln_b[2];
+  int ln_outs;
+  float ln_eps;
 };
 
-enum : int { EPI_GENERIC = 0, EPI_RESID = 1, EPI_ACT = 2, EPI_ROPE = 3, EPI_CONV = 4 };
+enum : int { EPI_GENERIC = 0, EPI_RESID = 1, EPI_ACT = 2, EPI_ROPE = 3, EPI_CONV = 4, EPI_RESID_LN = 5 };
 template <int EPI> struct EpiMask { static constexpr uint32_t value = 0xFFFFFFFFu; };
 template <> struct EpiMask<EPI_RESID> { static constexpr uint32_t value = F_BIAS | F_RESID_INPLACE; };
 template <> struct EpiMask<EPI_ACT> { static constexpr uint32_t value = F_BIAS | F_GELU | F_RELU; };
 template <> struct EpiMask<EPI_ROPE> { static constexpr uint32_t value = F_BIAS | F_ROPE; };
 template <> struct EpiMask<EPI_CONV> { static constexpr uint32_t value = F_BIAS | F_RELU | F_ADD0 | F_ADD1 | F_OUT2_RELU; };
+template <> struct EpiMask<EPI_RESID_LN> { static constexpr uint32_t value = F_BIAS | F_RESID_INPLACE; };
 
 struct ConvMaps {
   CUtensorMap out2, add0, add1;
@@ -71,15 +76,16 @@
   return EPI_GENERIC;
 }
 
-template <int BLOCK_N, bool TMA_STORE = false>
+template <int BLOCK_N, bool TMA_STORE = false, bool LN = false>
 struct Cfg {
   static constexpr int kStageA = BLOCK_M * BLOCK_K * 2;
   static constexpr int kStageB = BLOCK_N * BLOCK_K * 2;
   static constexpr int kStages = (BLOCK_N == 256) ? 4 : (BLOCK_N == 128) ? 6 : 8;
   static constexpr int kRing = kStages * (kStageA + kStageB);
-  static constexpr int kOutBuf = 64 * 128;
+  static constexpr int kOutBuf = LN ? 64 * 64 : 64 * 128;
   static constexpr int kStaging = TMA_STORE ? 2 * 2 * kOutBuf : 0;
-  static constexpr int kSmemBytes = kRing + kStaging + 1024  + 256  + (TMA_STORE ? 0 : (4 * 128 + 16) * 4) ;
+  static constexpr int kRecv = LN ? 2 * 4 * BLOCK_M * 8 : 0;
+  static constexpr int kSmemBytes = kRing + kStaging + kRecv + 1024  + 256  + (TMA_STORE ? 0 : (4 * 128 + 16) * 4) ;
   static_assert(kSmemBytes <= 227 * 1024, "shared memory of one CTA");
 };
 
@@ -97,32 +103,55 @@
   return fmaxf(x, 0.f) - fabsf(h);
 }
 
-template <int BLOCK_N, int EPI, bool PAIR, bool TMA_STORE>
+template <int BLOCK_N, int EPI, bool PAIR, bool TMA_STORE, int RC = 1>
 __device__ __forceinline__ void gemm_body(const CUtensorMap& tmap_a, const CUtensorMap& tmap_b, const CUtensorMap& tmap_o,
-                                          const ConvMaps* cm, const Params& p) {
+                                          const ConvMaps* cm, const Params& p, const CUtensorMap* tmap_o2 = nullptr,
+                                          const CUtensorMap* tmap_x = nullptr) {
   static_assert(EPI == EPI_CONV ? (TMA_STORE && (BLOCK_N == 256 || BLOCK_N == 128))
                                 : (!TMA_STORE || (BLOCK_N == 256 && EPI != EPI_GENERIC)),
                 "TMA-store epilogue: specialised projection epilogues on 128x256 tiles, the conv epilogue on 128x256 / 128x128");
-  using C = Cfg<BLOCK_N, TMA_STORE>;
+  static_assert((EPI == EPI_RESID_LN) == (RC > 1) && RC <= 4 && !(PAIR && RC > 1), "row clusters: the LayerNorm epilogue, 2 to 4 ranks");
+  constexpr bool kLN = EPI == EPI_RESID_LN;
+  constexpr bool kCluster = PAIR || RC > 1;
+  using C = Cfg<BLOCK_N, TMA_STORE, kLN>;
+  constexpr int kXBox = 64 * 128;
+  constexpr int kXBoxes = 2 * (BLOCK_N / 32);
+  constexpr int kXPerSlot = (C::kStageA + C::kStageB) / kXBox;
+  constexpr int kXEntries = (kXBoxes + kXPerSlot - 1) / kXPerSlot;
   extern __shared__ uint8_t smem_raw[];
   uint8_t* smem = reinterpret_cast<uint8_t*>((reinterpret_cast<uintptr_t>(smem_raw) + 1023) & ~uintptr_t(1023));
   uint8_t* smem_a = smem;
   uint8_t* smem_b = smem + C::kStages * C::kStageA;
   uint8_t* smem_o = smem + C::kRing;
-  uint64_t* bars = reinterpret_cast<uint64_t*>(smem + C::kRing + C::kStaging);
+  uint8_t* smem_recv = smem + C::kRing + C::kStaging;
+  uint64_t* bars = reinterpret_cast<uint64_t*>(smem + C::kRing + C::kStaging + C::kRecv);
   uint64_t* full_bar = bars;
   uint64_t* empty_bar = bars + C::kStages;
   uint64_t* add_bar = bars + 2 * C::kStages;
+  uint64_t* recv_bar = bars + 2 * C::kStages + 2;
   float* s_w4 = reinterpret_cast<float*>(reinterpret_cast<uint8_t*>(bars) + 256);
+  auto x_box = [&](int st, int k) {
+    return k < C::kStageA / kXBox ? ptx::smem_u32(smem_a + st * C::kStageA + k * kXBox)
+                                  : ptx::smem_u32(smem_b + st * C::kStageB + (k - C::kStageA / kXBox) * kXBox);
+  };
 
   const int warp = threadIdx.x >> 5, lane = threadIdx.x & 31;
-  const uint32_t rank = PAIR ? ptx::cluster_ctarank() : 0u;
+  const uint32_t rank = kCluster ? ptx::cluster_ctarank() : 0u;
   const int n_tiles = (p.N + BLOCK_N - 1) / BLOCK_N;
   const int m_tiles = (p.mode == 1) ? p.cB * p.tiles_y * p.tiles_x : (p.M + BLOCK_M - 1) / BLOCK_M;
   const int m_groups = PAIR ? (m_tiles + 1) / 2 : m_tiles;
-  const int total_items = m_groups * n_tiles;
-  const int first_item = PAIR ? blockIdx.x / 2 : blockIdx.x;
-  const int item_stride = PAIR ? gridDim.x / 2 : gridDim.x;
+  const int total_items = RC > 1 ? m_tiles : m_groups * n_tiles;
+  const int first_item = kCluster ? blockIdx.x / (PAIR ? 2 : RC) : blockIdx.x;
+  const int item_stride = kCluster ? gridDim.x / (PAIR ? 2 : RC) : gridDim.x;
+  auto item_tile = [&](int item, int& tm, int& tn) {
+    if constexpr (RC > 1) {
+      tm = item;
+      tn = int(rank);
+    } else {
+      tn = item % n_tiles;
+      tm = (item / n_tiles) * (PAIR ? 2 : 1) + int(rank);
+    }
+  };
 
   if (threadIdx.x == 0) {
     ptx::prefetch_tmap(&tmap_a);
@@ -130,7 +159,12 @@
     if constexpr (TMA_STORE) ptx::prefetch_tmap(&tmap_o);
     for (int s = 0; s < C::kStages; ++s) {
       ptx::mbar_init(ptx::smem_u32(&full_bar[s]), 1);
-      ptx::mbar_init(ptx::smem_u32(&empty_bar[s]), (PAIR ? 2 : 1) * kConsumerWarps);
+      ptx::mbar_init(ptx::smem_u32(&empty_bar[s]), (PAIR ? 2 : RC) * kConsumerWarps);
+    }
+    if constexpr (kLN) {
+      if (tmap_o2) ptx::prefetch_tmap(tmap_o2);
+      if (tmap_x) ptx::prefetch_tmap(tmap_x);
+      for (int i = 0; i < 4; ++i) ptx::mbar_init(ptx::smem_u32(&recv_bar[i]), 1);
     }
     if constexpr (EPI == EPI_CONV) {
       ptx::prefetch_tmap(&cm->out2);
@@ -145,7 +179,7 @@
     for (int i = threadIdx.x - 128; i < 4 * 128 + 4; i += 256) s_w4[i] = (i < 512) ? p.w4[i] : p.b4[i - 512];
   }
   __syncthreads();
-  if constexpr (PAIR) ptx::cluster_sync();
+  if constexpr (kCluster) ptx::cluster_sync();
   pdl::sync_with_predecessor();
 
   if (warp < 4) {
@@ -154,7 +188,8 @@
       int stage = 0;
       uint32_t phase = 0;
       for (int item = first_item; item < total_items; item += item_stride) {
-        const int tn = item % n_tiles, tm = (item / n_tiles) * (PAIR ? 2 : 1) + int(rank);
+        int tm, tn;
+        item_tile(item, tm, tn);
         int cb = 0, cy0 = 0, cx0 = 0;
         if (p.mode == 1) {
           cb = tm / (p.tiles_y * p.tiles_x);
@@ -175,6 +210,12 @@
             ptx::tma_load_4d(sa, &tmap_a, fb, cblk * BLOCK_K, cx0 + dx - 1, cy0 + dy - 1, cb);
             ka = cblk * BLOCK_K;
             kt = tap;
+          } else if constexpr (RC > 1) {
+            constexpr int kABox = (RC == 4) ? 32 : 64;
+            if (int(rank) * kABox < BLOCK_M)
+              ptx::tma_load_2d_mc(sa + rank * (kABox * BLOCK_K * 2), &tmap_a, fb, kb * BLOCK_K, tm * BLOCK_M + int(rank) * kABox,
+                                  uint16_t((1u << RC) - 1));
+            ka = kb * BLOCK_K;
           } else {
             ptx::tma_load_2d(sa, &tmap_a, fb, kb * BLOCK_K, tm * BLOCK_M);
             ka = kb * BLOCK_K;
@@ -186,6 +227,21 @@
             ptx::tma_load_3d(sb, &tmap_b, fb, ka, kt, tn * BLOCK_N);
           }
           if (++stage == C::kStages) { stage = 0; phase ^= 1; }
+        }
+        if constexpr (kLN) {
+          if (p.flags & F_RESID_INPLACE) {
+            for (int e = 0; e < kXEntries; ++e) {
+              const int n = (kXBoxes - e * kXPerSlot) < kXPerSlot ? (kXBoxes - e * kXPerSlot) : kXPerSlot;
+              ptx::mbar_wait(ptx::smem_u32(&empty_bar[stage]), phase ^ 1);
+              const uint32_t fb = ptx::smem_u32(&full_bar[stage]);
+              ptx::mbar_arrive_expect_tx(fb, uint32_t(n * kXBox));
+              for (int k = 0; k < n; ++k) {
+                const int b = e * kXPerSlot + k, half = b / (BLOCK_N / 32), c = b % (BLOCK_N / 32);
+                ptx::tma_load_2d(x_box(stage, k), tmap_x, fb, tn * BLOCK_N + c * 32, tm * BLOCK_M + half * 64);
+              }
+              if (++stage == C::kStages) { stage = 0; phase ^= 1; }
+            }
+          }
         }
       }
     }
@@ -205,6 +261,9 @@
         if constexpr (PAIR) {
           ptx::mbar_arrive_cluster(ptx::smem_u32(&empty_bar[s]), 0);
           ptx::mbar_arrive_cluster(ptx::smem_u32(&empty_bar[s]), 1);
+        } else if constexpr (RC > 1) {
+#pragma unroll
+          for (int r = 0; r < RC; ++r) ptx::mbar_arrive_cluster(ptx::smem_u32(&empty_bar[s]), uint32_t(r));
         } else {
           ptx::mbar_arrive(ptx::smem_u32(&empty_bar[s]));
         }
@@ -232,8 +291,12 @@
       if (flags & F_ADD0) ptx::tma_load_4d(b0, &cm->add0, bar, ch, bx, by, bb);
       if (flags & F_ADD1) ptx::tma_load_4d(out_buf(1), &cm->add1, bar, ch, bx, by, bb);
     };
+    const bool ln_resid = kLN && (flags & F_RESID_INPLACE) != 0;
+    uint32_t ln_tiles = 0;
+    auto ln_row = [&](int tm, int h) { return tm * BLOCK_M + wg * 64 + wq * 16 + (lane >> 2) + 8 * h; };
     for (int item = first_item; item < total_items; item += item_stride) {
-      const int tn = item % n_tiles, tm = (item / n_tiles) * (PAIR ? 2 : 1) + int(rank);
+      int tm, tn;
+      item_tile(item, tm, tn);
       if constexpr (EPI == EPI_CONV) {
         if (conv_add && conv_issuer) issue_addends(tm, tn * BLOCK_N);
       }
@@ -307,6 +370,154 @@
           }
         }
       }
+      if constexpr (kLN) {
+        float* xg = reinterpret_cast<float*>(p.out);
+        float sum[2] = {0.f, 0.f};
+        int xst[kXEntries];
+        uint32_t xph[kXEntries];
+        {
+          int st = stage;
+          uint32_t ph = phase;
+#pragma unroll
+          for (int e = 0; e < kXEntries; ++e) {
+            xst[e] = st;
+            xph[e] = ph;
+            if (++st == C::kStages) { st = 0; ph ^= 1; }
+          }
+        }
+        const uint32_t sw = lane >> 2;
+#pragma unroll
+        for (int c = 0; c < kNB / 4; ++c) {
+          const int b = wg * (kNB / 4) + c;
+          const int e = b / kXPerSlot;
+          int st = xst[0];
+          uint32_t ph = xph[0];
+#pragma unroll
+          for (int i = 1; i < kXEntries; ++i)
+            if (e == i) { st = xst[i]; ph = xph[i]; }
+          const uint32_t box = x_box(st, b - e * kXPerSlot);
+          if (ln_resid) ptx::mbar_wait(ptx::smem_u32(&full_bar[st]), ph);
+#pragma unroll
+          for (int h = 0; h < 2; ++h) {
+            const int row = ln_row(tm, h);
+            const uint32_t r = wq * 16 + (lane >> 2) + 8 * h;
+#pragma unroll
+            for (int jj = 0; jj < 4; ++jj) {
+              const int j = 4 * c + jj;
+              float& v0 = acc[4 * j + 2 * h];
+              float& v1 = acc[4 * j + 2 * h + 1];
+              if (ln_resid) {
+                const float2 xo = ptx::ld_shared_v2_f32(box + r * 128 + (((2 * jj + (q >> 1)) ^ sw) << 4) + (q & 1) * 8);
+                v0 += xo.x;
+                v1 += xo.y;
+              }
+              sum[h] += v0 + v1;
+              if (row < p.M) *reinterpret_cast<float2*>(xg + (long long)row * p.ldo + tn * BLOCK_N + 8 * j + 2 * q) = make_float2(v0, v1);
+            }
+          }
+        }
+        if (ln_resid) {
+          __syncwarp();
+#pragma unroll
+          for (int e = 0; e < kXEntries; ++e) release(xst[e]);
+          stage = xst[kXEntries - 1];
+          phase = xph[kXEntries - 1];
+          if (++stage == C::kStages) { stage = 0; phase ^= 1; }
+        }
+        float mean_r[2], m2_r[2];
+#pragma unroll
+        for (int h = 0; h < 2; ++h) {
+          sum[h] += __shfl_xor_sync(0xffffffffu, sum[h], 1);
+          sum[h] += __shfl_xor_sync(0xffffffffu, sum[h], 2);
+          mean_r[h] = sum[h] * (1.f / float(BLOCK_N));
+          float m2 = 0.f;
+#pragma unroll
+          for (int j = 0; j < kNB; ++j) {
+            const float a = acc[4 * j + 2 * h] - mean_r[h], b = acc[4 * j + 2 * h + 1] - mean_r[h];
+            m2 += a * a + b * b;
+          }
+          m2 += __shfl_xor_sync(0xffffffffu, m2, 1);
+          m2 += __shfl_xor_sync(0xffffffffu, m2, 2);
+          m2_r[h] = m2;
+        }
+        const uint32_t par = ln_tiles & 1;
+        const uint32_t rbar = ptx::smem_u32(&recv_bar[par * 2 + wg]);
+        const uint32_t slot = ptx::smem_u32(smem_recv) + par * (4 * BLOCK_M * 8);
+        if ((threadIdx.x & 127) == 0) ptx::mbar_arrive_expect_tx(rbar, uint32_t(RC * 64 * 8));
+        if (q == 0) {
+#pragma unroll
+          for (int h = 0; h < 2; ++h) {
+            const int row_in_tile = wg * 64 + wq * 16 + (lane >> 2) + 8 * h;
+#pragma unroll
+            for (int r = 0; r < RC; ++r)
+              ptx::st_async_v2_f32(slot + (rank * BLOCK_M + row_in_tile) * 8, rbar, uint32_t(r), mean_r[h], m2_r[h]);
+          }
+        }
+        ptx::mbar_wait(rbar, (ln_tiles >> 1) & 1);
+        ++ln_tiles;
+        float mean[2], rstd[2];
+#pragma unroll
+        for (int h = 0; h < 2; ++h) {
+          const int row_in_tile = wg * 64 + wq * 16 + (lane >> 2) + 8 * h;
+          float2 st[RC];
+#pragma unroll
+          for (int r = 0; r < RC; ++r) st[r] = ptx::ld_shared_v2_f32(slot + (r * BLOCK_M + row_in_tile) * 8);
+          float m = 0.f;
+#pragma unroll
+          for (int r = 0; r < RC; ++r) m += st[r].x;
+          m *= (1.f / float(RC));
+          float m2 = 0.f, d2 = 0.f;
+#pragma unroll
+          for (int r = 0; r < RC; ++r) {
+            m2 += st[r].y;
+            const float d = st[r].x - m;
+            d2 += d * d;
+          }
+          m2 += float(BLOCK_N) * d2;
+          mean[h] = m;
+          rstd[h] = rsqrtf(m2 / float(RC * BLOCK_N) + p.ln_eps);
+        }
+#pragma unroll
+        for (int j = 0; j < kNB; ++j)
+#pragma unroll
+          for (int h = 0; h < 2; ++h) {
+            acc[4 * j + 2 * h] = (acc[4 * j + 2 * h] - mean[h]) * rstd[h];
+            acc[4 * j + 2 * h + 1] = (acc[4 * j + 2 * h + 1] - mean[h]) * rstd[h];
+          }
+        const bool issuer = (threadIdx.x & 127) == 0;
+        for (int o = 0; o < p.ln_outs; ++o) {
+          const float* gg = o ? p.ln_g[1] : p.ln_g[0];
+          const float* bb = o ? p.ln_b[1] : p.ln_b[0];
+          const CUtensorMap* map = o ? tmap_o2 : &tmap_o;
+#pragma unroll
+          for (int c = 0; c < BLOCK_N / 32; ++c) {
+            const uint32_t buf = ptx::smem_u32(smem_o + (wg * 2 + (out_chunk & 1)) * C::kOutBuf);
+#pragma unroll
+            for (int jj = 0; jj < 4; ++jj) {
+              const int j = 4 * c + jj;
+              const int col = tn * BLOCK_N + 8 * j + 2 * q;
+              const float2 g2 = __ldg(reinterpret_cast<const float2*>(gg + col));
+              const float2 b2 = __ldg(reinterpret_cast<const float2*>(bb + col));
+#pragma unroll
+              for (int h = 0; h < 2; ++h) {
+                const uint32_t row = wq * 16 + (lane >> 2) + 8 * h;
+                const float y0 = acc[4 * j + 2 * h] * g2.x + b2.x;
+                const float y1 = acc[4 * j + 2 * h + 1] * g2.y + b2.y;
+                ptx::st_shared_b32(buf + row * 64 + ((uint32_t(jj) ^ ((row >> 1) & 3)) << 4) + q * 4, pack_bf16x2(y0, y1));
+              }
+            }
+            ptx::fence_proxy_async();
+            if (issuer) ptx::bulk_wait_group_read<0>();
+            ptx::named_bar_sync(1 + wg, 128);
+            if (issuer) {
+              ptx::tma_store_2d(map, buf, tn * BLOCK_N + c * 32, tm * BLOCK_M + wg * 64);
+              ptx::bulk_commit_group();
+            }
+            ++out_chunk;
+          }
+        }
+        continue;
+      }
       if (flags & F_ROPE) {
 #pragma unroll
         for (int cb = 0; cb < BLOCK_N / 32; ++cb) {
@@ -488,7 +699,7 @@
       if ((threadIdx.x & 127) == 0) ptx::bulk_wait_group<0>();
     }
   }
-  if constexpr (PAIR) ptx::cluster_sync();
+  if constexpr (kCluster) ptx::cluster_sync();
 }
 
 template <int BLOCK_N, int EPI, bool PAIR, bool TMA_STORE>
@@ -498,6 +709,14 @@
   gemm_body<BLOCK_N, EPI, PAIR, TMA_STORE>(tmap_a, tmap_b, tmap_o, nullptr, p);
 }
 
+template <int RC>
+__global__ void __launch_bounds__(kNumThreads, 1)
+resid_ln_kernel(const __grid_constant__ CUtensorMap tmap_a, const __grid_constant__ CUtensorMap tmap_b,
+                const __grid_constant__ CUtensorMap tmap_y0, const __grid_constant__ CUtensorMap tmap_y1,
+                const __grid_constant__ CUtensorMap tmap_x, const Params p) {
+  gemm_body<256, EPI_RESID_LN, false, true, RC>(tmap_a, tmap_b, tmap_y0, nullptr, p, &tmap_y1, &tmap_x);
+}
+
 template <int BLOCK_N, bool PAIR>
 __global__ void __launch_bounds__(kNumThreads, 1)
 conv_kernel(const __grid_constant__ CUtensorMap tmap_a, const __grid_constant__ CUtensorMap tmap_b,
diff --git a/dust3r_b200/csrc/sm90_ptx.cuh b/dust3r_b200/csrc/sm90_ptx.cuh
--- a/dust3r_b200/csrc/sm90_ptx.cuh
+++ b/dust3r_b200/csrc/sm90_ptx.cuh
@@ -100,6 +100,12 @@
   asm volatile(
       "cp.async.bulk.tensor.3d.shared::cluster.global.mbarrier::complete_tx::bytes.multicast::cluster [%0], [%1, {%3, %4, %5}], [%2], %6;"
       ::"r"(dst), "l"(reinterpret_cast<uint64_t>(tmap)), "r"(bar), "r"(c0), "r"(c1), "r"(c2), "h"(mask)
+      : "memory");
+}
+__device__ __forceinline__ void tma_load_2d_mc(uint32_t dst, const void* tmap, uint32_t bar, int c0, int c1, uint16_t mask) {
+  asm volatile(
+      "cp.async.bulk.tensor.2d.shared::cluster.global.mbarrier::complete_tx::bytes.multicast::cluster [%0], [%1, {%3, %4}], [%2], %5;"
+      ::"r"(dst), "l"(reinterpret_cast<uint64_t>(tmap)), "r"(bar), "r"(c0), "r"(c1), "h"(mask)
       : "memory");
 }
 
@@ -145,6 +151,20 @@
       "mbarrier.arrive.shared::cluster.b64 _, [raddr];\n"
       "}\n" ::"r"(bar), "r"(rank) : "memory");
 }
+__device__ __forceinline__ void st_async_v2_f32(uint32_t addr, uint32_t bar, uint32_t rank, float a, float b) {
+  asm volatile(
+      "{\n"
+      ".reg .b32 raddr, rbar;\n"
+      "mapa.shared::cluster.u32 raddr, %0, %2;\n"
+      "mapa.shared::cluster.u32 rbar, %1, %2;\n"
+      "st.async.shared::cluster.mbarrier::complete_tx::bytes.v2.f32 [raddr], {%3, %4}, [rbar];\n"
+      "}\n" ::"r"(addr), "r"(bar), "r"(rank), "f"(a), "f"(b) : "memory");
+}
+__device__ __forceinline__ float2 ld_shared_v2_f32(uint32_t addr) {
+  float2 v;
+  asm volatile("ld.shared.v2.f32 {%0, %1}, [%2];" : "=f"(v.x), "=f"(v.y) : "r"(addr) : "memory");
+  return v;
+}
 
 __device__ __forceinline__ float ex2_approx(float x) { float y; asm("ex2.approx.ftz.f32 %0, %1;" : "=f"(y) : "f"(x)); return y; }
 __device__ __forceinline__ float rcp_approx(float x) { float y; asm("rcp.approx.ftz.f32 %0, %1;" : "=f"(y) : "f"(x)); return y; }
diff --git a/include/dust3r_b200.h b/include/dust3r_b200.h
--- a/include/dust3r_b200.h
+++ b/include/dust3r_b200.h
@@ -139,6 +139,10 @@
                   void* out2_dev, int32_t M, int32_t N, int32_t K, int64_t ldo, uint32_t flags,
                   const float* rope_cos_dev, const float* rope_sin_dev, int32_t rope_cols, int32_t tokens_per_img,
                   int32_t grid_w, void* stream);
+
+int d3r_gemm_resid_ln(const void* A_dev, const void* B_dev, float* x_dev, const float* bias_dev, int32_t M, int32_t N, int32_t K,
+                      int32_t resid, const float* g0_dev, const float* b0_dev, void* y0_dev, const float* g1_dev,
+                      const float* b1_dev, void* y1_dev, float eps, void* stream);
 
 int d3r_conv3x3_bf16(const void* x_nhwc_dev, const void* w_packed_dev, void* out_dev, const float* bias_dev,
                      const void* add0_dev, const void* add1_dev, void* out2_dev, int32_t B, int32_t H, int32_t W,
```
